# slp-rl/aero

Measured on NVIDIA H100. Metric: audio-seconds/sec forward, higher is better.
Workload: dtype f16 tensor-core operands and activation storage (10-bit mantissa = tf32), fp32 accumulate / norm inputs / cell state

## Files before the change

### aero_b200/csrc/tapgemm.cuh

```cuda
#pragma once
#include <cuda.h>
#include "common.cuh"

namespace aero {
struct TapGemmArgs {
    const void* a1;
    const void* a2;
    const void* w;
    const float* bias;
    const float* addend_fn;
    const float* colscale;
    const void* residual;
    const float* samp_affine;
    void* out;
    double* stats;
    aero_tapgemm_params p;
    int ntaps;
    int tiles_t;
    int ldw;
    int vec_a;
    int vec_o;
    int vec_o8;
    uint32_t dv_mul[3], dv_shr[3];
    int direct_f16;
    int direct_f32;
    int last_tile;
};
constexpr int kBM = 128;
constexpr int kMaxStages = 8;
constexpr int kMaxBN = 128;
constexpr int kEpiWarps = 8;
constexpr int kThreads = 128 + 32 * kEpiWarps;
constexpr int kATileBytes = kBM * 128;

struct TcShared {
    uint64_t full[kMaxStages];
    uint64_t empty[kMaxStages];
    float stats[kEpiWarps][8][2];
    float part[kEpiWarps][4][2];
    alignas(16) float stage[kEpiWarps][32][20];
};

using KernelFn = void (*)(CUtensorMap, CUtensorMap, CUtensorMap, TapGemmArgs, int, int, int);
int tapgemm_simt_launch(const TapGemmArgs& g, cudaStream_t st);
int tapgemm_tc_launch(const TapGemmArgs& g, cudaStream_t st);
bool tapgemm_tc_eligible(const aero_tapgemm_params& p);
}
```

### aero_b200/csrc/tapgemm_tc.cu

```cuda
#include <cuda.h>
#include <mutex>
#include <unordered_map>
#include <string>
#include <cstring>
#include <cstdlib>

#include "tapgemm.cuh"
#include "tc_common.cuh"

namespace aero {

KernelFn tapgemm_tc_kernels_bn32(bool f16a, bool f16o, int amode, bool res, bool stats);
KernelFn tapgemm_tc_kernels_bn64(bool f16a, bool f16o, int amode, bool res, bool stats);
KernelFn tapgemm_tc_kernels_bn96(bool f16a, bool f16o, int amode, bool res, bool stats);
KernelFn tapgemm_tc_kernels_bn128(bool f16a, bool f16o, int amode, bool res, bool stats);

typedef CUresult (*EncodeTiledFn)(CUtensorMap*, CUtensorMapDataType, cuuint32_t, void*, const cuuint64_t*, const cuuint64_t*,
                                  const cuuint32_t*, const cuuint32_t*, CUtensorMapInterleave, CUtensorMapSwizzle,
                                  CUtensorMapL2promotion, CUtensorMapFloatOOBfill);

static EncodeTiledFn get_encode() {
    static EncodeTiledFn fn = nullptr;
    static std::once_flag once;
    std::call_once(once, [] {
        void* p = nullptr;
        cudaDriverEntryPointQueryResult qres;
        if (cudaGetDriverEntryPoint("cuTensorMapEncodeTiled", &p, cudaEnableDefault, &qres) == cudaSuccess &&
            qres == cudaDriverEntryPointSuccess)
            fn = reinterpret_cast<EncodeTiledFn>(p);
    });
    return fn;
}

struct MapKey {
    const void* base;
    uint64_t d[4], s[3];
    uint32_t box[4], rank, swz, pad_;
    bool operator==(const MapKey& o) const { return std::memcmp(this, &o, sizeof(MapKey)) == 0; }
};
struct MapKeyHash {
    size_t operator()(const MapKey& k) const {
        const uint64_t* w = reinterpret_cast<const uint64_t*>(&k);
        size_t h = 1469598103934665603ull;
        for (size_t i = 0; i < sizeof(MapKey) / 8; ++i) h = (h ^ w[i]) * 1099511628211ull;
        return h;
    }
};

int encode_map(CUtensorMap* out, const void* base, uint32_t rank, const uint64_t* dims, const uint64_t* strides_bytes,
               const uint32_t* box, int swizzle_mode, int elem_bytes) {
    static std::mutex mu;
    static std::unordered_map<MapKey, CUtensorMap, MapKeyHash> cache;
    MapKey key;
    std::memset(&key, 0, sizeof(key));
    key.base = base;
    key.rank = rank;
    key.swz = (uint32_t)swizzle_mode | ((uint32_t)elem_bytes << 8);
    for (uint32_t i = 0; i < rank; ++i) { key.d[i] = dims[i]; key.box[i] = box[i]; }
    for (uint32_t i = 0; i + 1 < rank; ++i) key.s[i] = strides_bytes[i];
    {
        std::lock_guard<std::mutex> lk(mu);
        auto it = cache.find(key);
        if (it != cache.end()) { *out = it->second; return AERO_OK; }
    }
    EncodeTiledFn enc = get_encode();
    if (!enc) { set_error("cuTensorMapEncodeTiled not available from the driver"); return AERO_ERR_UNSUPPORTED; }
    cuuint64_t gd[4];
    cuuint64_t gs[3];
    cuuint32_t bx[4], es[4];
    for (uint32_t i = 0; i < rank; ++i) { gd[i] = dims[i]; bx[i] = box[i]; es[i] = 1; }
    for (uint32_t i = 0; i + 1 < rank; ++i) gs[i] = strides_bytes[i];
    CUresult r = enc(out, elem_bytes == 2 ? CU_TENSOR_MAP_DATA_TYPE_FLOAT16 : CU_TENSOR_MAP_DATA_TYPE_FLOAT32, rank, const_cast<void*>(base), gd, gs, bx, es,
                     CU_TENSOR_MAP_INTERLEAVE_NONE,
                     swizzle_mode == 2 ? CU_TENSOR_MAP_SWIZZLE_64B : CU_TENSOR_MAP_SWIZZLE_128B,
                     CU_TENSOR_MAP_L2_PROMOTION_L2_256B,
                     CU_TENSOR_MAP_FLOAT_OOB_FILL_NONE);
    if (r != CUDA_SUCCESS) {
        set_error("cuTensorMapEncodeTiled failed (%d): rank %u dims %llu %llu %llu %llu", (int)r, rank,
                  (unsigned long long)dims[0], (unsigned long long)dims[1], (unsigned long long)(rank > 2 ? dims[2] : 0),
                  (unsigned long long)(rank > 3 ? dims[3] : 0));
        return AERO_ERR_INVALID;
    }
    std::lock_guard<std::mutex> lk(mu);
    if (cache.size() > 4096) cache.clear();
    cache.emplace(key, *out);
    return AERO_OK;
}

static int pick_bn(int N) {
    const int ntiles = (N + kMaxBN - 1) / kMaxBN;
    const int per = (N + ntiles - 1) / ntiles;
    return (per + 31) & ~31;
}

static int tc_fixed_smem(int N, int BN) { return (int)sizeof(TcShared) + cdiv(N, BN) * BN * 4 + kBM * (BN + 4) * 4 + 1024; }
static int tc_stages(int N, int BN) {
    if (N > (1 << 20)) return 0;
    const int st = (227 * 1024 - tc_fixed_smem(N, BN)) / (kATileBytes + BN * 128);
    return st > kMaxStages ? kMaxStages : st;
}

bool tapgemm_tc_eligible(const aero_tapgemm_params& p) {
    const bool f16 = (p.flags & AERO_TG_A_F16) != 0;
    const int q = f16 ? 8 : 4;
    if (p.mode == AERO_TAPS_MIX)
        return p.w_sb == 0 && p.C1 % q == 0 && p.C2 == 0 && p.a1_st % q == 0 && p.a1_sb % q == 0 && p.N >= 8 &&
               p.stats_mode == 0 && !p.glu && p.F_out == 1 && p.F_in == 1 && tc_stages(p.N, pick_bn(p.N)) >= 2;
    if (p.w_sb != 0) return false;
    if (p.act == AERO_ACT_TANH) return false;
    if (p.act == AERO_ACT_LEAKY && (p.stats_mode != 0 || p.r_sb != 0 || p.r_sf != 0 || p.r_st != 0))
        return false;
    if (tc_stages(p.N, pick_bn(p.N)) < 2) return false;
    if (p.N < 8) return false;
    const int K = p.C1 + p.C2;
    if (K < 8 || (p.C1 % q) || (p.C2 % q)) return false;
    auto ok_strides = [q](int64_t sb, int64_t sf, int64_t st) { return sb % q == 0 && sf % q == 0 && st % q == 0 && st > 0; };
    if (p.C1 && !ok_strides(p.a1_sb, p.a1_sf, p.a1_st)) return false;
    if (p.C2 && !ok_strides(p.a2_sb, p.a2_sf, p.a2_st)) return false;
    if (p.stats_mode == 1) {
        const int Nout = p.glu ? p.N / 2 : p.N;
        if (p.groups < 1 || Nout % p.groups) return false;
        const int gw = Nout / p.groups;
        const int bn = pick_bn(p.N);
        if (gw % 8 || (p.glu ? bn / 2 : bn) / gw + 2 > 8) return false;
    }
    return true;
}

static int make_a_map(CUtensorMap* m, const void* base, int C, const aero_tapgemm_params& p, int64_t sb, int64_t sf, int64_t st, int esz) {
    uint64_t dims[4] = {(uint64_t)C, (uint64_t)p.T_in, (uint64_t)p.F_in, (uint64_t)p.B};
    int64_t s1 = st, s2 = sf, s3 = sb;
    if (s2 <= 0) s2 = s1 * p.T_in;
    if (s3 <= 0) s3 = s2 * p.F_in;
    uint64_t strides[3] = {(uint64_t)s1 * esz, (uint64_t)s2 * esz, (uint64_t)s3 * esz};
    uint32_t box[4] = {(uint32_t)(128 / esz), (uint32_t)kBM, 1, 1};
    return encode_map(m, base, 4, dims, strides, box, 0, esz);
}

struct TcKnobs {
    int direct_f32 = -1, direct_f16 = -1, stages = -1;
    TcKnobs() {
        auto rd = [](const char* name, int& v) { if (const char* e = getenv(name)) v = atoi(e); };
        rd("AERO_TC_DIRECT_F32", direct_f32); rd("AERO_TC_DIRECT_F16", direct_f16); rd("AERO_TC_STAGES", stages);
    }
};
static const TcKnobs& knobs() { static const TcKnobs k; return k; }

int tapgemm_tc_launch(const TapGemmArgs& g0, cudaStream_t st) {
    const TcKnobs& kn = knobs();
    TapGemmArgs g = g0;
    const aero_tapgemm_params& p = g.p;
    const bool f16a = p.precision == 2, f16o = (p.flags & AERO_TG_OUT_F16) != 0;
    const int esz = f16a ? 2 : 4, kBKc = 128 / esz;
    const int K = p.C1 + p.C2;
    const int BN = pick_bn(p.N);
    const int nslab = (p.mode == AERO_TAPS_CONVT) ? p.kf : p.kf * p.kt;
    CUtensorMap mA1, mA2, mW;
    int rc;
    const bool mix = p.mode == AERO_TAPS_MIX;
    if (mix) {
        uint64_t dims[3] = {(uint64_t)p.T, (uint64_t)p.C1, (uint64_t)p.B};
        uint64_t strides[2] = {(uint64_t)p.a1_st * esz, (uint64_t)(p.a1_sb > 0 ? p.a1_sb : (int64_t)p.a1_st * p.C1) * esz};
        uint32_t box[3] = {(uint32_t)(f16a ? 64 : 32), (uint32_t)kBKc, 1};
        if ((rc = encode_map(&mA1, g.a1, 3, dims, strides, box, 0, esz)) != AERO_OK) return rc;
    } else if (p.C1) { if ((rc = make_a_map(&mA1, g.a1, p.C1, p, p.a1_sb, p.a1_sf, p.a1_st, esz)) != AERO_OK) return rc; }
    if (p.C2) { if ((rc = make_a_map(&mA2, g.a2, p.C2, p, p.a2_sb, p.a2_sf, p.a2_st, esz)) != AERO_OK) return rc; }
    if (!p.C1) mA1 = mA2;
    if (!p.C2) mA2 = mA1;
    {
        const uint64_t npad = (uint64_t)((p.N + 3) & ~3);
        const uint64_t kp = f16a ? (uint64_t)((K + 7) & ~7) : (uint64_t)K;
        uint64_t dims[3] = {(uint64_t)K, npad, (uint64_t)nslab};
        uint64_t strides[2] = {kp * esz, kp * npad * esz};
        uint32_t box[3] = {(uint32_t)kBKc, (uint32_t)BN, 1};
        if ((rc = encode_map(&mW, g.w, 3, dims, strides, box, 0, esz)) != AERO_OK) return rc;
    }
    g.tiles_t = cdiv(p.T, kBM);
    g.direct_f32 = 0;
    g.direct_f16 = 2;
    if (kn.direct_f32 >= 0) g.direct_f32 = kn.direct_f32;
    if (kn.direct_f16 >= 0) g.direct_f16 = kn.direct_f16;
    const int64_t tiles = (int64_t)p.B * p.F_out * g.tiles_t;
    if (tiles > 2147483647LL) { set_error("aero_tapgemm_fwd: too many tiles"); return AERO_ERR_INVALID; }
    {
        const uint32_t divs[3] = {(uint32_t)cdiv(p.N, BN), (uint32_t)g.tiles_t, (uint32_t)p.F_out};
        for (int i = 0; i < 3; ++i) {
            uint32_t s = 0;
            while ((1ull << s) < divs[i]) ++s;
            const uint64_t two = 1ull << (31 + s);
            g.dv_mul[i] = (uint32_t)((two + divs[i] - 1) / divs[i]);
            g.dv_shr[i] = 31 + s;
        }
    }
    const int stage_bytes = kATileBytes + BN * 128;
    const int fixed = tc_fixed_smem(p.N, BN);
    int kStages = tc_stages(p.N, BN);
    if (kStages < 2) {
        set_error("aero_tapgemm_fwd(wgmma): N = %d leaves no shared memory for the pipeline", p.N);
        return AERO_ERR_UNSUPPORTED;
    }
    if (kn.stages >= 2 && kn.stages < kStages) kStages = kn.stages;
    const size_t smem = (size_t)kStages * stage_bytes + fixed;
    const int amode = p.glu ? 3 : (p.act == AERO_ACT_LEAKY ? 4 : p.act);
    if (p.glu && p.act != AERO_ACT_NONE) { set_error("aero_tapgemm_fwd(wgmma): GLU with an activation is not supported"); return AERO_ERR_UNSUPPORTED; }
    const bool res = g.residual != nullptr, stats = p.stats_mode != 0;
    const KernelFn kern = BN == 32 ? tapgemm_tc_kernels_bn32(f16a, f16o, amode, res, stats)
                        : BN == 64 ? tapgemm_tc_kernels_bn64(f16a, f16o, amode, res, stats)
                        : BN == 96 ? tapgemm_tc_kernels_bn96(f16a, f16o, amode, res, stats)
                                   : tapgemm_tc_kernels_bn128(f16a, f16o, amode, res, stats);
    if (!kern) {
        set_error("aero_tapgemm_fwd(wgmma): epilogue (act %d, residual %d, stats %d) is not built for operands %s / outputs %s",
                  amode, (int)res, (int)stats, f16a ? "f16" : "tf32", f16o ? "f16" : "f32");
        return AERO_ERR_UNSUPPORTED;
    }
    cudaFuncSetAttribute(kern, cudaFuncAttributeMaxDynamicSharedMemorySize, 227 * 1024);
    static int num_sms = 0;
    if (num_sms == 0) {
        int dev = 0;
        cudaGetDevice(&dev);
        cudaDeviceGetAttribute(&num_sms, cudaDevAttrMultiProcessorCount, dev);
    }
    const int n_tiles = cdiv(p.N, BN);
    const int64_t tiles_total = tiles * n_tiles;
    if (tiles_total > 2147483647LL) { set_error("aero_tapgemm_fwd: too many tiles"); return AERO_ERR_INVALID; }
    const int64_t want = num_sms;
    g.last_tile = (int)tiles_total - 1;
    dim3 grid((unsigned)(tiles_total < want ? tiles_total : want));
    kern<<<grid, kThreads, smem, st>>>(mA1, mA2, mW, g, kStages, n_tiles, (int)tiles_total);
    return check_launch("aero_tapgemm_fwd(wgmma)");
}

}
```

### aero_b200/csrc/tapgemm_tc_kernel.cuh

```cuda
#pragma once
#include <cuda.h>
#include <type_traits>

#include "tapgemm.cuh"
#include "tc_common.cuh"


namespace aero {

template <bool F16A> struct OperandKind { static constexpr int kBK = F16A ? 64 : 32; };

struct TapIter {
    int fi, dt, slab;
};
__device__ __forceinline__ bool tap_geometry(const aero_tapgemm_params& p, int tap, int fo, TapIter& it) {
    if (p.mode == AERO_TAPS_CONV) {
        const int jf = tap / p.kt, jt = tap - jf * p.kt;
        it.fi = fo * p.stride_f + jf - p.pad_f;
        it.dt = jt * p.dil_t - p.pad_t;
        it.slab = tap;
    } else {
        const int fof = fo + p.f_out_offset;
        it.fi = fof / p.stride_f - tap;
        it.dt = 0;
        it.slab = fof % p.stride_f + tap * p.stride_f;
    }
    return it.fi >= 0 && it.fi < p.F_in;
}

struct TileCoord {
    int b, fo, t0, n0, n_iters;
};
__device__ __forceinline__ int fast_div(int n, uint32_t mul, uint32_t shr) {
    return (int)(((uint64_t)(uint32_t)n * mul) >> shr);
}
__device__ __forceinline__ int valid_taps(const aero_tapgemm_params& p, int fo, int ntaps) {
    if (p.mode == AERO_TAPS_CONV) {
        const int base = fo * p.stride_f - p.pad_f;
        const int lo = max(0, -base), hi = min(p.kf - 1, p.F_in - 1 - base);
        return max(0, hi - lo + 1) * p.kt;
    }
    const int a = (fo + p.f_out_offset) / p.stride_f;
    const int lo = max(0, a - p.F_in + 1), hi = min(ntaps - 1, a);
    return max(0, hi - lo + 1);
}
__device__ __forceinline__ TileCoord tile_coord(const TapGemmArgs& g, int tile, int n_tiles, int BN, int nch1, int nch2) {
    const aero_tapgemm_params& p = g.p;
    TileCoord c;
    if (p.flags & AERO_TG_REVERSE) tile = g.last_tile - tile;
    const int mt = fast_div(tile, g.dv_mul[0], g.dv_shr[0]), nt = tile - mt * n_tiles;
    const int row = fast_div(mt, g.dv_mul[1], g.dv_shr[1]), tt = mt - row * g.tiles_t;
    c.b = fast_div(row, g.dv_mul[2], g.dv_shr[2]);
    c.fo = row - c.b * p.F_out;
    c.t0 = tt * kBM;
    c.n0 = nt * BN;
    c.n_iters = (p.mode == AERO_TAPS_MIX) ? nch1 : valid_taps(p, c.fo, g.ntaps) * (nch1 + nch2);
    return c;
}

template <int AMODE>
__device__ __forceinline__ void epilogue_stage_a(const uint32_t (&r)[16], uint32_t stg_row, uint32_t sbias) {
    float4 bv[4];
#pragma unroll
    for (int j = 0; j < 4; ++j) bv[j] = lds128(sbias + 16 * j);
#pragma unroll
    for (int j = 0; j < 16; j += 4) {
        float v[4] = {__uint_as_float(r[j]) + bv[j / 4].x, __uint_as_float(r[j + 1]) + bv[j / 4].y,
                      __uint_as_float(r[j + 2]) + bv[j / 4].z, __uint_as_float(r[j + 3]) + bv[j / 4].w};
#pragma unroll
        for (int u = 0; u < 4; ++u) {
            if (AMODE == 1) v[u] = gelu_exact(v[u]);
            else if (AMODE == 2) v[u] = fmaxf(v[u], 0.f);
            else if (AMODE == 4) v[u] = leaky_f(v[u]);
        }
        if (AMODE == 3) {
            sts64(stg_row + (j / 2) * 4, v[0] * sigmoid_f(v[1]), v[2] * sigmoid_f(v[3]));
        } else {
            sts128(stg_row + j * 4, make_float4(v[0], v[1], v[2], v[3]));
        }
    }
}

template <int AMODE, bool RES, bool STATS, typename TO>
__device__ __forceinline__ void epilogue_fast_tile(TcShared* sh, const TapGemmArgs& g, const TileCoord& tc, uint32_t tacc, int BN, int q,
                                                   int ew, int lane, int Nout, int gw, int c_start, int c_step, uint32_t sbias) {
    const aero_tapgemm_params& p = g.p;
    constexpr int CNT = (AMODE == 3) ? 8 : 16;
    constexpr int LPR = CNT / 4;
    constexpr int RPI = 32 / LPR;
    const uint32_t stg = smem_u32(&sh->stage[ew][0][0]);
    const bool rnd = (p.flags & 1) && sizeof(TO) == 4;
    float sa = 1.f, sb = 0.f;
    if (g.samp_affine) { sa = g.samp_affine[2 * tc.b]; sb = g.samp_affine[2 * tc.b + 1]; }
    const int cq = lane % LPR, ro = lane / LPR;
    const int row0 = tc.t0 + q * 32;
    const int rows = min(32, p.T - row0);
    const int g_lo = ((AMODE == 3) ? tc.n0 >> 1 : tc.n0) / gw;
    TO* const obase = static_cast<TO*>(g.out) + (int64_t)tc.b * p.o_sb + (int64_t)tc.fo * p.o_sf + (int64_t)row0 * p.o_st;
    const TO* const rbase = RES ? static_cast<const TO*>(g.residual) + (int64_t)tc.b * p.r_sb + (int64_t)tc.fo * p.r_sf + (int64_t)row0 * p.r_st : nullptr;
    const float* const adp = g.addend_fn ? g.addend_fn + (int64_t)tc.fo * Nout : nullptr;
    for (int c0 = c_start; c0 < BN; c0 += c_step) {
        const int nb = tc.n0 + c0;
        if (nb >= p.N) break;
        uint32_t r[16];
        if (tc.n_iters > 0) {
            acc_ld16(tacc + 4u * (uint32_t)c0, r);
        } else {
#pragma unroll
            for (int j = 0; j < 16; ++j) r[j] = 0u;
        }
        epilogue_stage_a<AMODE>(r, stg + (uint32_t)lane * 80u, sbias + (uint32_t)nb * 4u);
        __syncwarp();
        const int no0 = (AMODE == 3) ? nb >> 1 : nb;
        const int nn = no0 + 4 * cq;
        float ls = 0.f, lq = 0.f;
        if (nn < Nout) {
            float4 ad = make_float4(0.f, 0.f, 0.f, 0.f);
            const bool has_ad = adp != nullptr, affine = g.samp_affine != nullptr;
            if (has_ad) ad = *reinterpret_cast<const float4*>(adp + nn);
            uint32_t sp = stg + (uint32_t)(ro * 80 + cq * 16);
            TO* op = obase + (int64_t)ro * p.o_st + nn;
            const TO* rp = RES ? rbase + (int64_t)ro * p.r_st + nn : nullptr;
            const int64_t ostep = (int64_t)RPI * p.o_st, rstep = (int64_t)RPI * p.r_st;
#pragma unroll 2
            for (int rr = ro; rr < rows; rr += RPI) {
                float4 x = lds128(sp);
                sp += RPI * 80;
                if (has_ad) { x.x += ad.x; x.y += ad.y; x.z += ad.z; x.w += ad.w; }
                if (RES) {
                    const float4 rs = ld4(rp);
                    x.x += rs.x; x.y += rs.y; x.z += rs.z; x.w += rs.w;
                    rp += rstep;
                }
                if (affine) { x.x = fmaf(x.x, sa, sb); x.y = fmaf(x.y, sa, sb); x.z = fmaf(x.z, sa, sb); x.w = fmaf(x.w, sa, sb); }
                if (rnd) { x.x = round_tf32_rna(x.x); x.y = round_tf32_rna(x.y); x.z = round_tf32_rna(x.z); x.w = round_tf32_rna(x.w); }
                if (STATS) {
                    if (sizeof(TO) == 2) {
                        x.x = stored(x.x, op); x.y = stored(x.y, op); x.z = stored(x.z, op); x.w = stored(x.w, op);
                    }
                    ls += (x.x + x.y) + (x.z + x.w);
                    lq += (x.x * x.x + x.y * x.y) + (x.z * x.z + x.w * x.w);
                }
                st4(op, x);
                op += ostep;
            }
        }
        if (STATS) {
            const int g_first = no0 / gw, g_last = (min(no0 + CNT, Nout) - 1) / gw;
            if (g_first == g_last) {
                const float a = warp_sum(ls), c = warp_sum(lq);
                if (lane == 0) { sh->stats[ew][g_first - g_lo][0] += a; sh->stats[ew][g_first - g_lo][1] += c; }
            } else {
                for (int o = LPR; o < 32; o <<= 1) { ls += __shfl_xor_sync(0xffffffffu, ls, o); lq += __shfl_xor_sync(0xffffffffu, lq, o); }
                if (lane < LPR) { sh->part[ew][lane][0] = ls; sh->part[ew][lane][1] = lq; }
                __syncwarp();
                if (lane == 0) {
                    for (int u = 0; u < LPR; ++u) {
                        const int nq = no0 + 4 * u;
                        if (nq < Nout) {
                            sh->stats[ew][nq / gw - g_lo][0] += sh->part[ew][u][0];
                            sh->stats[ew][nq / gw - g_lo][1] += sh->part[ew][u][1];
                        }
                    }
                }
            }
        }
        __syncwarp();
    }
}

template <int AMODE, bool RES, bool STATS, typename TO>
__device__ __forceinline__ void epilogue_direct(TcShared* sh, const TapGemmArgs& g, const TileCoord& tc, uint32_t tacc, int BN, int q, int ew,
                                                int lane, int Nout, int gw, int c_start, int c_step, uint32_t sbias) {
    const aero_tapgemm_params& p = g.p;
    constexpr int CNT = (AMODE == 3) ? 8 : 16;
    constexpr bool F16 = sizeof(TO) == 2;
    const int t = tc.t0 + q * 32 + lane;
    const bool row_ok = t < p.T;
    TO* const orow = static_cast<TO*>(g.out) + (int64_t)tc.b * p.o_sb + (int64_t)tc.fo * p.o_sf + (int64_t)t * p.o_st;
    const TO* const rrow = RES ? static_cast<const TO*>(g.residual) + (int64_t)tc.b * p.r_sb + (int64_t)tc.fo * p.r_sf + (int64_t)t * p.r_st : nullptr;
    const float* const adp = g.addend_fn ? g.addend_fn + (int64_t)tc.fo * Nout : nullptr;
    float sa = 1.f, sb = 0.f;
    const bool affine = g.samp_affine != nullptr;
    if (affine) { sa = g.samp_affine[2 * tc.b]; sb = g.samp_affine[2 * tc.b + 1]; }
    const bool rnd = (p.flags & 1) && !F16;
    const int g_lo = ((AMODE == 3) ? tc.n0 >> 1 : tc.n0) / gw;
    int cur_g = -1;
    float ssum = 0.f, ssq = 0.f;
    for (int c0 = c_start; c0 < BN; c0 += c_step) {
        const int nb = tc.n0 + c0;
        if (nb >= p.N) break;
        uint32_t r[16];
        if (tc.n_iters > 0) {
            acc_ld16(tacc + 4u * (uint32_t)c0, r);
        } else {
#pragma unroll
            for (int j = 0; j < 16; ++j) r[j] = 0u;
        }
        float v[16];
#pragma unroll
        for (int j = 0; j < 16; ++j) v[j] = __uint_as_float(r[j]);
        {
            float4 bv[4];
#pragma unroll
            for (int j = 0; j < 4; ++j) bv[j] = lds128(sbias + (uint32_t)nb * 4u + 16u * j);
#pragma unroll
            for (int j = 0; j < 4; ++j) { v[4 * j] += bv[j].x; v[4 * j + 1] += bv[j].y; v[4 * j + 2] += bv[j].z; v[4 * j + 3] += bv[j].w; }
        }
        float o[CNT];
        if (AMODE == 3) {
#pragma unroll
            for (int j = 0; j < 8; ++j) o[j] = v[2 * j] * sigmoid_f(v[2 * j + 1]);
        } else {
#pragma unroll
            for (int j = 0; j < 16; ++j)
                o[j] = (AMODE == 1) ? gelu_exact(v[j]) : (AMODE == 2) ? fmaxf(v[j], 0.f) : (AMODE == 4) ? leaky_f(v[j]) : v[j];
        }
        const int no0 = (AMODE == 3) ? nb >> 1 : nb;
        const int n_ok = min(CNT, Nout - no0);
        if (row_ok) {
            if (adp) {
#pragma unroll
                for (int j = 0; j < CNT; j += 4)
                    if (j < n_ok) {
                        const float4 a = __ldg(reinterpret_cast<const float4*>(adp + no0 + j));
                        o[j] += a.x; o[j + 1] += a.y; o[j + 2] += a.z; o[j + 3] += a.w;
                    }
            }
            if (RES) {
#pragma unroll
                for (int j = 0; j < CNT; j += 4)
                    if (j < n_ok) {
                        const float4 a = ld4(rrow + no0 + j);
                        o[j] += a.x; o[j + 1] += a.y; o[j + 2] += a.z; o[j + 3] += a.w;
                    }
            }
            if (affine) {
#pragma unroll
                for (int j = 0; j < CNT; ++j) o[j] = fmaf(o[j], sa, sb);
            }
            if (rnd) {
#pragma unroll
                for (int j = 0; j < CNT; ++j) o[j] = round_tf32_rna(o[j]);
            }
            if (F16 && STATS) {
#pragma unroll
                for (int j = 0; j < CNT; ++j) o[j] = stored(o[j], orow);
            }
            if (F16) {
#pragma unroll
                for (int j = 0; j < CNT; j += 8)
                    if (j < n_ok) {
                        uint4 u;
                        u.x = pack_half2_sat(o[j], o[j + 1]); u.y = pack_half2_sat(o[j + 2], o[j + 3]);
                        u.z = pack_half2_sat(o[j + 4], o[j + 5]); u.w = pack_half2_sat(o[j + 6], o[j + 7]);
                        *reinterpret_cast<uint4*>(orow + no0 + j) = u;
                    }
            } else {
#pragma unroll
                for (int j = 0; j < CNT; j += 4)
                    if (j < n_ok) *reinterpret_cast<float4*>(orow + no0 + j) = make_float4(o[j], o[j + 1], o[j + 2], o[j + 3]);
            }
        }
        if (STATS) {
#pragma unroll
            for (int j = 0; j < CNT; j += 4) {
                if (j < n_ok) {
                    const int gi = (no0 + j) / gw;
                    if (gi != cur_g) {
                        if (cur_g >= 0) {
                            const float a = warp_sum(ssum), c = warp_sum(ssq);
                            if (lane == 0) { sh->stats[ew][cur_g - g_lo][0] += a; sh->stats[ew][cur_g - g_lo][1] += c; }
                        }
                        cur_g = gi; ssum = 0.f; ssq = 0.f;
                    }
                    if (row_ok) {
                        ssum += (o[j] + o[j + 1]) + (o[j + 2] + o[j + 3]);
                        ssq += (o[j] * o[j] + o[j + 1] * o[j + 1]) + (o[j + 2] * o[j + 2] + o[j + 3] * o[j + 3]);
                    }
                }
            }
        }
    }
    if (STATS && cur_g >= 0) {
        const float a = warp_sum(ssum), c = warp_sum(ssq);
        if (lane == 0) { sh->stats[ew][cur_g - g_lo][0] += a; sh->stats[ew][cur_g - g_lo][1] += c; }
    }
}

template <int BN, bool F16A>
__device__ __forceinline__ void tile_mainloop(TcShared* sh, uint8_t* smem, int& stage, uint32_t& phase, const int kStages, const int stage_bytes,
                                              const int n_iters, const bool mix, const int wg, float* acc, const int ldacc) {
    float d[BN / 2];
    const int tid = threadIdx.x & 127, wl = tid >> 5, lane = tid & 31;
    int prev = -1;
    for (int i = 0; i < n_iters; ++i) {
        mbar_wait(&sh->full[stage], phase);
        const uint32_t sa = smem_u32(smem + stage * stage_bytes);
        const uint64_t db = make_desc_sw128(sa + kATileBytes);
        wgmma_fence();
        if (mix && F16A) {
            if constexpr (F16A) {
                const uint32_t sw = sa + (uint32_t)wg * 8192u;
                const uint64_t da = (uint64_t)((sw >> 4) & 0x3FFF) | ((uint64_t)(8192 >> 4) << 16) | ((uint64_t)(1024 >> 4) << 32) | ((uint64_t)1 << 62);
#pragma unroll
                for (int k = 0; k < 4; ++k) Wgmma<BN, true, 1>::ss(d, da + (uint64_t)(k * (2048 >> 4)), db + 2 * k, (i > 0 || k > 0) ? 1u : 0u);
            }
        } else if (mix) {
            if constexpr (!F16A) {
                const int m = wg * 64 + wl * 16 + (lane >> 2), c = lane & 3;
#pragma unroll
                for (int k = 0; k < 4; ++k) {
                    uint32_t a[4];
#pragma unroll
                    for (int u = 0; u < 4; ++u) {
                        const int mm = m + (u & 1) * 8, kk = 8 * k + c + (u >> 1) * 4;
                        const uint32_t addr = sa + (uint32_t)((mm >> 5) * 4096 + kk * 128 + ((((mm & 31) >> 2) ^ (kk & 7)) << 4) + ((mm & 3) << 2));
                        asm volatile("ld.shared.b32 %0, [%1];" : "=r"(a[u]) : "r"(addr));
                    }
                    Wgmma<BN, false, 0>::rs(d, a, db + 2 * k, (i > 0 || k > 0) ? 1u : 0u);
                }
            }
        } else {
            const uint64_t da = make_desc_sw128(sa + (uint32_t)wg * (64 * 128));
#pragma unroll
            for (int k = 0; k < 4; ++k)
                Wgmma<BN, F16A, 0>::ss(d, da + 2 * k, db + 2 * k, (i > 0 || k > 0) ? 1u : 0u);
        }
        wgmma_commit();
        wgmma_wait<1>();
        if (prev >= 0 && tid == 0) mbar_arrive(&sh->empty[prev]);
        prev = stage;
        if (++stage == kStages) { stage = 0; phase ^= 1; }
    }
    wgmma_wait<0>();
    if (prev >= 0 && tid == 0) mbar_arrive(&sh->empty[prev]);
    float* row = acc + (wg * 64 + wl * 16 + (lane >> 2)) * ldacc + 2 * (lane & 3);
#pragma unroll
    for (int j = 0; j < BN / 8; ++j) {
        *reinterpret_cast<float2*>(row + 8 * j) = make_float2(d[4 * j], d[4 * j + 1]);
        *reinterpret_cast<float2*>(row + 8 * ldacc + 8 * j) = make_float2(d[4 * j + 2], d[4 * j + 3]);
    }
}

template <int BN, int AMODE, bool RES, bool STATS, bool F16A, bool F16O>
__global__ void __launch_bounds__(kThreads, 1)
tapgemm_tc_kernel(const __grid_constant__ CUtensorMap mapA1, const __grid_constant__ CUtensorMap mapA2,
                  const __grid_constant__ CUtensorMap mapW, const TapGemmArgs g, const int kStages, const int n_tiles,
                  const int tiles_total) {
    extern __shared__ uint8_t smem_raw[];
    uint8_t* smem = reinterpret_cast<uint8_t*>((reinterpret_cast<uintptr_t>(smem_raw) + 1023) & ~(uintptr_t)1023);
    constexpr int stage_bytes = kATileBytes + BN * 128;
    TcShared* sh = reinterpret_cast<TcShared*>(smem + kStages * stage_bytes);
    float* const sbias_f = reinterpret_cast<float*>(sh + 1);
    const uint32_t sbias = smem_u32(sbias_f);
    float* const acc = sbias_f + n_tiles * BN;
    constexpr int ldacc = BN + 4;

    using TO = typename std::conditional<F16O, __half, float>::type;
    constexpr int kBKc = OperandKind<F16A>::kBK;
    const aero_tapgemm_params& p = g.p;
    const int warp = threadIdx.x >> 5, lane = threadIdx.x & 31;
    const int nch1 = (p.C1 + kBKc - 1) / kBKc, nch2 = (p.C2 + kBKc - 1) / kBKc;
    const bool mix = p.mode == AERO_TAPS_MIX;

    for (int i = threadIdx.x; i < n_tiles * BN; i += kThreads) sbias_f[i] = (g.bias && i < g.p.N) ? g.bias[i] : 0.f;
    if (threadIdx.x == 0) {
        for (int s = 0; s < kStages; ++s) { mbar_init(&sh->full[s], 1); mbar_init(&sh->empty[s], 2); }
        asm volatile("fence.mbarrier_init.release.cluster;" ::: "memory");
        for (int w = 0; w < kEpiWarps; ++w)
            for (int i = 0; i < 8; ++i) { sh->stats[w][i][0] = 0.f; sh->stats[w][i][1] = 0.f; }
    }
    __syncthreads();

    if (warp == 0) {
        if (lane == 0) {
            asm volatile("prefetch.tensormap [%0];" ::"l"(&mapA1) : "memory");
            asm volatile("prefetch.tensormap [%0];" ::"l"(&mapW) : "memory");
            int stage = 0;
            uint32_t phase = 0;
            const uint32_t tx = (uint32_t)stage_bytes;
            int ptl = 0;
            for (int tile = blockIdx.x; tile < tiles_total; tile += gridDim.x, ++ptl) {
                const TileCoord c = tile_coord(g, tile, n_tiles, BN, nch1, nch2);
                if (mix) {
                    for (int kc = 0; kc < nch1; ++kc) {
                        mbar_wait(&sh->empty[stage], phase ^ 1);
                        uint8_t* sa = smem + stage * stage_bytes;
                        mbar_expect_tx(&sh->full[stage], tx);
                        constexpr int kBoxM = F16A ? 64 : 32;
#pragma unroll
                        for (int j = 0; j < 128 / kBoxM; ++j)
                            tma_load_3d(sa + j * (kATileBytes / (128 / kBoxM)), &mapA1, &sh->full[stage], c.t0 + kBoxM * j, kc * kBKc, c.b);
                        tma_load_3d(sa + kATileBytes, &mapW, &sh->full[stage], kc * kBKc, c.n0, 0);
                        if (++stage == kStages) { stage = 0; phase ^= 1; }
                    }
                    continue;
                }
                for (int tap = 0; tap < g.ntaps; ++tap) {
                    TapIter it;
                    if (!tap_geometry(p, tap, c.fo, it)) continue;
                    for (int src = 0; src < 2; ++src) {
                        const int nch = src ? nch2 : nch1;
                        const CUtensorMap* mA = src ? &mapA2 : &mapA1;
                        const int kw0 = src ? p.C1 : 0;
                        for (int kc = 0; kc < nch; ++kc) {
                            mbar_wait(&sh->empty[stage], phase ^ 1);
                            uint8_t* sa = smem + stage * stage_bytes;
                            mbar_expect_tx(&sh->full[stage], tx);
                            tma_load_4d(sa, mA, &sh->full[stage], kc * kBKc, c.t0 + it.dt, it.fi, c.b);
                            tma_load_3d(sa + kATileBytes, &mapW, &sh->full[stage], kw0 + kc * kBKc, c.n0, it.slab);
                            if (++stage == kStages) { stage = 0; phase ^= 1; }
                        }
                    }
                }
            }
        }
    } else if (warp >= 4) {
        const int wg = (warp >> 2) - 1;
        const int ew = warp - 4;
        const int q = 2 * wg + (warp & 1);
        const int grp = (warp >> 1) & 1;
        const int m = q * 32 + lane;
        const int Nout = p.glu ? p.N / 2 : p.N;
        const int gw = (p.stats_mode == 1) ? Nout / p.groups : Nout;
        const bool rnd = (p.flags & 1) && !F16O;
        const int c_start = grp * 16, c_step = 32;
        const bool fast = !mix && g.vec_o && !g.colscale && (p.stats_mode == 0 || gw % 4 == 0);
        int stage = 0, local = 0;
        uint32_t phase = 0;
        for (int tile = blockIdx.x; tile < tiles_total; tile += gridDim.x, ++local) {
            const TileCoord tc = tile_coord(g, tile, n_tiles, BN, nch1, nch2);
            const int b = tc.b, fo = tc.fo, t0 = tc.t0, n0 = tc.n0, n_iters = tc.n_iters;
            tile_mainloop<BN, F16A>(sh, smem, stage, phase, kStages, stage_bytes, n_iters, mix, wg, acc, ldacc);
            warpgroup_sync(1 + wg);
            const uint32_t tacc = smem_u32(acc + m * ldacc);
            const int t = t0 + m;
            const bool row_ok = t < p.T;
            float sa = 1.f, sb = 0.f;
            if (g.samp_affine) { sa = g.samp_affine[2 * b]; sb = g.samp_affine[2 * b + 1]; }
            TO* op = static_cast<TO*>(g.out) + (int64_t)b * p.o_sb + (int64_t)fo * p.o_sf + (int64_t)t * p.o_st;
            const TO* rp = g.residual ? static_cast<const TO*>(g.residual) + (int64_t)b * p.r_sb + (int64_t)fo * p.r_sf + (int64_t)t * p.r_st : nullptr;
            const float* csp = g.colscale ? g.colscale + (int64_t)b * p.cs_sb + (int64_t)t * p.cs_st : nullptr;
            const float* adp = g.addend_fn ? g.addend_fn + (int64_t)fo * Nout : nullptr;
            int cur_g = -1;
            float ssum = 0.f, ssq = 0.f;
            const int g_lo = (p.glu ? n0 >> 1 : n0) / gw;

            if (mix) {
                const float gate = (row_ok && g.colscale) ? g.colscale[(int64_t)b * p.cs_sb + t] : 1.f;
                TO* ob = static_cast<TO*>(g.out) + (int64_t)b * p.o_sb + t;
                for (int c0 = c_start; c0 < BN; c0 += c_step) {
                    uint32_t r[16];
                    acc_ld16(tacc + 4u * (uint32_t)c0, r);
                    if (row_ok) {
#pragma unroll
                        for (int j = 0; j < 16; ++j) {
                            const int n = n0 + c0 + j;
                            if (n < p.N) {
                                float x = __uint_as_float(r[j]) * gate;
                                if (rnd) x = round_tf32_rna(x);
                                stf(ob + (int64_t)n * p.o_st, x);
                            }
                        }
                    }
                }
            } else if (fast && (F16O ? (g.vec_o8 && (g.direct_f16 == 1 || (g.direct_f16 == 2 && AMODE == 3))) : g.direct_f32)) {
                epilogue_direct<AMODE, RES, STATS, TO>(sh, g, tc, tacc, BN, q, ew, lane, Nout, gw, c_start, c_step, sbias);
            } else if (fast) {
                epilogue_fast_tile<AMODE, RES, STATS, TO>(sh, g, tc, tacc, BN, q, ew, lane, Nout, gw, c_start, c_step, sbias);
            } else {
                for (int c0 = 0; c0 < (grp == 0 ? BN : 0); c0 += 16) {
                    uint32_t r[16];
                    if (n_iters > 0) {
                        acc_ld16(tacc + 4u * (uint32_t)c0, r);
                    } else {
#pragma unroll
                        for (int j = 0; j < 16; ++j) r[j] = 0u;
                    }
                    const int nb = n0 + c0;
                    if (nb >= p.N) continue;
                    float v[16];
#pragma unroll
                    for (int j = 0; j < 16; ++j) {
                        const int n = nb + j;
                        float x = __uint_as_float(r[j]);
                        if (row_ok && n < p.N) {
                            x += sbias_f[n];
                            if (csp) x *= csp[n];
                            if (p.act == AERO_ACT_GELU) x = gelu_exact(x);
                            else if (p.act == AERO_ACT_RELU) x = fmaxf(x, 0.f);
                            else if (AMODE == 4) x = leaky_f(x);
                        }
                        v[j] = x;
                    }
                    float o[16];
                    int no0, cnt;
                    if (p.glu) {
                        no0 = nb >> 1;
                        cnt = 8;
#pragma unroll
                        for (int j = 0; j < 8; ++j) o[j] = v[2 * j] * sigmoid_f(v[2 * j + 1]);
                    } else {
                        no0 = nb;
                        cnt = 16;
#pragma unroll
                        for (int j = 0; j < 16; ++j) o[j] = v[j];
                    }
#pragma unroll
                    for (int sub = 0; sub < 2; ++sub) {
                        if (sub * 8 >= cnt) break;
                        const int ns = no0 + sub * 8;
                        if (p.stats_mode != 0 && ns < Nout) {
                            const int gi = ns / gw;
                            if (gi != cur_g) {
                                if (cur_g >= 0) {
                                    const float a = warp_sum(ssum), c = warp_sum(ssq);
                                    if (lane == 0) { sh->stats[ew][cur_g - g_lo][0] = a; sh->stats[ew][cur_g - g_lo][1] = c; }
                                }
                                cur_g = gi; ssum = 0.f; ssq = 0.f;
                            }
                        }
#pragma unroll
                        for (int j = 0; j < 8; ++j) {
                            const int jj = sub * 8 + j;
                            const int nn = no0 + jj;
                            if (row_ok && nn < Nout) {
                                float x = o[jj];
                                if (adp) x += adp[nn];
                                if (rp) x += ldf(rp + nn);
                                x = x * sa + sb;
                                if (rnd) x = round_tf32_rna(x);
                                x = stored(x, op);
                                o[jj] = x;
                                ssum += x;
                                ssq += x * x;
                            }
                        }
                    }
                    if (row_ok) {
#pragma unroll
                        for (int j = 0; j < 16; ++j)
                            if (j < cnt && no0 + j < Nout) stf(op + no0 + j, o[j]);
                    }
                }
                if (p.stats_mode != 0 && cur_g >= 0) {
                    const float a = warp_sum(ssum), c = warp_sum(ssq);
                    if (lane == 0) { sh->stats[ew][cur_g - g_lo][0] = a; sh->stats[ew][cur_g - g_lo][1] = c; }
                }
            }
            warpgroup_sync(1 + wg);
            if (p.stats_mode != 0) {
                __syncwarp();
                if (lane < 8) {
                    const float a = sh->stats[ew][lane][0], c = sh->stats[ew][lane][1];
                    const int gi = g_lo + lane;
                    const int ngroups = (p.stats_mode == 1) ? p.groups : 1;
                    if (gi < ngroups && (a != 0.f || c != 0.f)) {
                        const int64_t slot = (p.stats_mode == 1) ? ((int64_t)b * p.groups + gi) : ((int64_t)b * p.F_out + fo);
                        atomicAdd(&g.stats[2 * slot], (double)a);
                        atomicAdd(&g.stats[2 * slot + 1], (double)c);
                    }
                    sh->stats[ew][lane][0] = 0.f;
                    sh->stats[ew][lane][1] = 0.f;
                }
                __syncwarp();
            }
        }
    }
}



template <int BN, bool F16A, bool F16O>
static KernelFn pick_kernel(int amode, bool res, bool stats) {
#define AERO_TC_K(A, R, S) tapgemm_tc_kernel<BN, A, R, S, F16A, F16O>
    if (amode == 4) return (res || stats) ? nullptr : AERO_TC_K(4, false, false);
    if constexpr (!F16A && !F16O) {
        static const KernelFn table[4][2][2] = {
            {{AERO_TC_K(0, false, false), AERO_TC_K(0, false, true)}, {AERO_TC_K(0, true, false), AERO_TC_K(0, true, true)}},
            {{AERO_TC_K(1, false, false), AERO_TC_K(1, false, true)}, {AERO_TC_K(1, true, false), AERO_TC_K(1, true, true)}},
            {{AERO_TC_K(2, false, false), AERO_TC_K(2, false, true)}, {AERO_TC_K(2, true, false), AERO_TC_K(2, true, true)}},
            {{AERO_TC_K(3, false, false), AERO_TC_K(3, false, true)}, {AERO_TC_K(3, true, false), AERO_TC_K(3, true, true)}}};
        return table[amode][res][stats];
    } else if constexpr (F16O) {
        if (stats) return (amode == 0 && !res) ? AERO_TC_K(0, false, true) : nullptr;
        if (res) return amode == 0 ? AERO_TC_K(0, true, false) : nullptr;
        switch (amode) {
            case 0: return AERO_TC_K(0, false, false);
            case 1: return AERO_TC_K(1, false, false);
            case 2: return AERO_TC_K(2, false, false);
            default: return AERO_TC_K(3, false, false);
        }
    } else {
        if (res) return nullptr;
        if (stats) return amode == 0 ? AERO_TC_K(0, false, true) : nullptr;
        switch (amode) {
            case 0: return AERO_TC_K(0, false, false);
            case 1: return AERO_TC_K(1, false, false);
            case 2: return AERO_TC_K(2, false, false);
            default: return AERO_TC_K(3, false, false);
        }
    }
#undef AERO_TC_K
}

template <int BN>
static KernelFn pick_kernel_bn(bool f16a, bool f16o, int amode, bool res, bool stats) {
    return f16a ? (f16o ? pick_kernel<BN, true, true>(amode, res, stats) : pick_kernel<BN, true, false>(amode, res, stats))
                : (f16o ? pick_kernel<BN, false, true>(amode, res, stats) : pick_kernel<BN, false, false>(amode, res, stats));
}

}
```

### aero_b200/csrc/wgmma.cuh

```cuda
#pragma once
#include <cstdint>

namespace aero {

__device__ __forceinline__ void wgmma_fence() { asm volatile("wgmma.fence.sync.aligned;" ::: "memory"); }
__device__ __forceinline__ void wgmma_commit() { asm volatile("wgmma.commit_group.sync.aligned;" ::: "memory"); }
template <int PENDING>
__device__ __forceinline__ void wgmma_wait() { asm volatile("wgmma.wait_group.sync.aligned %0;" ::"n"(PENDING) : "memory"); }

template <int ROWB>
__device__ __forceinline__ uint64_t make_desc_kmajor(uint32_t saddr) {
    return (uint64_t)((saddr >> 4) & 0x3FFF) | ((uint64_t)1 << 16) | ((uint64_t)((ROWB * 8) >> 4) << 32) |
           ((uint64_t)(ROWB == 128 ? 1 : 2) << 62);
}
__device__ __forceinline__ uint64_t make_desc_sw128(uint32_t saddr) { return make_desc_kmajor<128>(saddr); }

template <int N, bool F16, int TA> struct Wgmma;

template <int TA> struct Wgmma<16, true, TA> {
    static __device__ __forceinline__ void ss(float (&d)[8], uint64_t da, uint64_t db, uint32_t acc) {
        asm volatile("{\n\t.reg .pred p;\n\tsetp.ne.b32 p, %10, 0;\n\t"
                     "wgmma.mma_async.sync.aligned.m64n16k16.f32.f16.f16 {%0, %1, %2, %3, %4, %5, %6, %7}, %8, %9, p, 1, 1, %11, 0;\n\t}"
            : "+f"(d[0]), "+f"(d[1]), "+f"(d[2]), "+f"(d[3]), "+f"(d[4]), "+f"(d[5]), "+f"(d[6]), "+f"(d[7])
            : "l"(da), "l"(db), "r"(acc), "n"(TA));
    }
};
template <> struct Wgmma<16, false, 0> {
    static __device__ __forceinline__ void ss(float (&d)[8], uint64_t da, uint64_t db, uint32_t acc) {
        asm volatile("{\n\t.reg .pred p;\n\tsetp.ne.b32 p, %10, 0;\n\t"
                     "wgmma.mma_async.sync.aligned.m64n16k8.f32.tf32.tf32 {%0, %1, %2, %3, %4, %5, %6, %7}, %8, %9, p, 1, 1;\n\t}"
            : "+f"(d[0]), "+f"(d[1]), "+f"(d[2]), "+f"(d[3]), "+f"(d[4]), "+f"(d[5]), "+f"(d[6]), "+f"(d[7])
            : "l"(da), "l"(db), "r"(acc));
    }
    static __device__ __forceinline__ void rs(float (&d)[8], const uint32_t (&a)[4], uint64_t db, uint32_t acc) {
        asm volatile("{\n\t.reg .pred p;\n\tsetp.ne.b32 p, %13, 0;\n\t"
                     "wgmma.mma_async.sync.aligned.m64n16k8.f32.tf32.tf32 {%0, %1, %2, %3, %4, %5, %6, %7}, {%8, %9, %10, %11}, %12, p, 1, 1;\n\t}"
            : "+f"(d[0]), "+f"(d[1]), "+f"(d[2]), "+f"(d[3]), "+f"(d[4]), "+f"(d[5]), "+f"(d[6]), "+f"(d[7])
            : "r"(a[0]), "r"(a[1]), "r"(a[2]), "r"(a[3]), "l"(db), "r"(acc));
    }
};

template <int TA> struct Wgmma<32, true, TA> {
    static __device__ __forceinline__ void ss(float (&d)[16], uint64_t da, uint64_t db, uint32_t acc) {
        asm volatile("{\n\t.reg .pred p;\n\tsetp.ne.b32 p, %18, 0;\n\t"
                     "wgmma.mma_async.sync.aligned.m64n32k16.f32.f16.f16 {%0, %1, %2, %3, %4, %5, %6, %7, %8, %9, %10, %11, %12, %13, %14, %15}, %16, %17, p, 1, 1, %19, 0;\n\t}"
            : "+f"(d[0]), "+f"(d[1]), "+f"(d[2]), "+f"(d[3]), "+f"(d[4]), "+f"(d[5]), "+f"(d[6]), "+f"(d[7]),
              "+f"(d[8]), "+f"(d[9]), "+f"(d[10]), "+f"(d[11]), "+f"(d[12]), "+f"(d[13]), "+f"(d[14]), "+f"(d[15])
            : "l"(da), "l"(db), "r"(acc), "n"(TA));
    }
};
template <> struct Wgmma<32, false, 0> {
    static __device__ __forceinline__ void ss(float (&d)[16], uint64_t da, uint64_t db, uint32_t acc) {
        asm volatile("{\n\t.reg .pred p;\n\tsetp.ne.b32 p, %18, 0;\n\t"
                     "wgmma.mma_async.sync.aligned.m64n32k8.f32.tf32.tf32 {%0, %1, %2, %3, %4, %5, %6, %7, %8, %9, %10, %11, %12, %13, %14, %15}, %16, %17, p, 1, 1;\n\t}"
            : "+f"(d[0]), "+f"(d[1]), "+f"(d[2]), "+f"(d[3]), "+f"(d[4]), "+f"(d[5]), "+f"(d[6]), "+f"(d[7]),
              "+f"(d[8]), "+f"(d[9]), "+f"(d[10]), "+f"(d[11]), "+f"(d[12]), "+f"(d[13]), "+f"(d[14]), "+f"(d[15])
            : "l"(da), "l"(db), "r"(acc));
    }
    static __device__ __forceinline__ void rs(float (&d)[16], const uint32_t (&a)[4], uint64_t db, uint32_t acc) {
        asm volatile("{\n\t.reg .pred p;\n\tsetp.ne.b32 p, %21, 0;\n\t"
                     "wgmma.mma_async.sync.aligned.m64n32k8.f32.tf32.tf32 {%0, %1, %2, %3, %4, %5, %6, %7, %8, %9, %10, %11, %12, %13, %14, %15}, {%16, %17, %18, %19}, %20, p, 1, 1;\n\t}"
            : "+f"(d[0]), "+f"(d[1]), "+f"(d[2]), "+f"(d[3]), "+f"(d[4]), "+f"(d[5]), "+f"(d[6]), "+f"(d[7]),
              "+f"(d[8]), "+f"(d[9]), "+f"(d[10]), "+f"(d[11]), "+f"(d[12]), "+f"(d[13]), "+f"(d[14]), "+f"(d[15])
            : "r"(a[0]), "r"(a[1]), "r"(a[2]), "r"(a[3]), "l"(db), "r"(acc));
    }
};

template <int TA> struct Wgmma<48, true, TA> {
    static __device__ __forceinline__ void ss(float (&d)[24], uint64_t da, uint64_t db, uint32_t acc) {
        asm volatile("{\n\t.reg .pred p;\n\tsetp.ne.b32 p, %26, 0;\n\t"
                     "wgmma.mma_async.sync.aligned.m64n48k16.f32.f16.f16 {%0, %1, %2, %3, %4, %5, %6, %7, %8, %9, %10, %11, %12, %13, %14, %15, %16, %17, %18, %19, %20, %21, %22, %23}, %24, %25, p, 1, 1, %27, 0;\n\t}"
            : "+f"(d[0]), "+f"(d[1]), "+f"(d[2]), "+f"(d[3]), "+f"(d[4]), "+f"(d[5]), "+f"(d[6]), "+f"(d[7]),
              "+f"(d[8]), "+f"(d[9]), "+f"(d[10]), "+f"(d[11]), "+f"(d[12]), "+f"(d[13]), "+f"(d[14]), "+f"(d[15]),
              "+f"(d[16]), "+f"(d[17]), "+f"(d[18]), "+f"(d[19]), "+f"(d[20]), "+f"(d[21]), "+f"(d[22]), "+f"(d[23])
            : "l"(da), "l"(db), "r"(acc), "n"(TA));
    }
};
template <> struct Wgmma<48, false, 0> {
    static __device__ __forceinline__ void ss(float (&d)[24], uint64_t da, uint64_t db, uint32_t acc) {
        asm volatile("{\n\t.reg .pred p;\n\tsetp.ne.b32 p, %26, 0;\n\t"
                     "wgmma.mma_async.sync.aligned.m64n48k8.f32.tf32.tf32 {%0, %1, %2, %3, %4, %5, %6, %7, %8, %9, %10, %11, %12, %13, %14, %15, %16, %17, %18, %19, %20, %21, %22, %23}, %24, %25, p, 1, 1;\n\t}"
            : "+f"(d[0]), "+f"(d[1]), "+f"(d[2]), "+f"(d[3]), "+f"(d[4]), "+f"(d[5]), "+f"(d[6]), "+f"(d[7]),
              "+f"(d[8]), "+f"(d[9]), "+f"(d[10]), "+f"(d[11]), "+f"(d[12]), "+f"(d[13]), "+f"(d[14]), "+f"(d[15]),
              "+f"(d[16]), "+f"(d[17]), "+f"(d[18]), "+f"(d[19]), "+f"(d[20]), "+f"(d[21]), "+f"(d[22]), "+f"(d[23])
            : "l"(da), "l"(db), "r"(acc));
    }
    static __device__ __forceinline__ void rs(float (&d)[24], const uint32_t (&a)[4], uint64_t db, uint32_t acc) {
        asm volatile("{\n\t.reg .pred p;\n\tsetp.ne.b32 p, %29, 0;\n\t"
                     "wgmma.mma_async.sync.aligned.m64n48k8.f32.tf32.tf32 {%0, %1, %2, %3, %4, %5, %6, %7, %8, %9, %10, %11, %12, %13, %14, %15, %16, %17, %18, %19, %20, %21, %22, %23}, {%24, %25, %26, %27}, %28, p, 1, 1;\n\t}"
            : "+f"(d[0]), "+f"(d[1]), "+f"(d[2]), "+f"(d[3]), "+f"(d[4]), "+f"(d[5]), "+f"(d[6]), "+f"(d[7]),
              "+f"(d[8]), "+f"(d[9]), "+f"(d[10]), "+f"(d[11]), "+f"(d[12]), "+f"(d[13]), "+f"(d[14]), "+f"(d[15]),
              "+f"(d[16]), "+f"(d[17]), "+f"(d[18]), "+f"(d[19]), "+f"(d[20]), "+f"(d[21]), "+f"(d[22]), "+f"(d[23])
            : "r"(a[0]), "r"(a[1]), "r"(a[2]), "r"(a[3]), "l"(db), "r"(acc));
    }
};

template <int TA> struct Wgmma<64, true, TA> {
    static __device__ __forceinline__ void ss(float (&d)[32], uint64_t da, uint64_t db, uint32_t acc) {
        asm volatile("{\n\t.reg .pred p;\n\tsetp.ne.b32 p, %34, 0;\n\t"
                     "wgmma.mma_async.sync.aligned.m64n64k16.f32.f16.f16 {%0, %1, %2, %3, %4, %5, %6, %7, %8, %9, %10, %11, %12, %13, %14, %15, %16, %17, %18, %19, %20, %21, %22, %23, %24, %25, %26, %27, %28, %29, %30, %31}, %32, %33, p, 1, 1, %35, 0;\n\t}"
            : "+f"(d[0]), "+f"(d[1]), "+f"(d[2]), "+f"(d[3]), "+f"(d[4]), "+f"(d[5]), "+f"(d[6]), "+f"(d[7]),
              "+f"(d[8]), "+f"(d[9]), "+f"(d[10]), "+f"(d[11]), "+f"(d[12]), "+f"(d[13]), "+f"(d[14]), "+f"(d[15]),
              "+f"(d[16]), "+f"(d[17]), "+f"(d[18]), "+f"(d[19]), "+f"(d[20]), "+f"(d[21]), "+f"(d[22]), "+f"(d[23]),
              "+f"(d[24]), "+f"(d[25]), "+f"(d[26]), "+f"(d[27]), "+f"(d[28]), "+f"(d[29]), "+f"(d[30]), "+f"(d[31])
            : "l"(da), "l"(db), "r"(acc), "n"(TA));
    }
};
template <> struct Wgmma<64, false, 0> {
    static __device__ __forceinline__ void ss(float (&d)[32], uint64_t da, uint64_t db, uint32_t acc) {
        asm volatile("{\n\t.reg .pred p;\n\tsetp.ne.b32 p, %34, 0;\n\t"
                     "wgmma.mma_async.sync.aligned.m64n64k8.f32.tf32.tf32 {%0, %1, %2, %3, %4, %5, %6, %7, %8, %9, %10, %11, %12, %13, %14, %15, %16, %17, %18, %19, %20, %21, %22, %23, %24, %25, %26, %27, %28, %29, %30, %31}, %32, %33, p, 1, 1;\n\t}"
            : "+f"(d[0]), "+f"(d[1]), "+f"(d[2]), "+f"(d[3]), "+f"(d[4]), "+f"(d[5]), "+f"(d[6]), "+f"(d[7]),
              "+f"(d[8]), "+f"(d[9]), "+f"(d[10]), "+f"(d[11]), "+f"(d[12]), "+f"(d[13]), "+f"(d[14]), "+f"(d[15]),
              "+f"(d[16]), "+f"(d[17]), "+f"(d[18]), "+f"(d[19]), "+f"(d[20]), "+f"(d[21]), "+f"(d[22]), "+f"(d[23]),
              "+f"(d[24]), "+f"(d[25]), "+f"(d[26]), "+f"(d[27]), "+f"(d[28]), "+f"(d[29]), "+f"(d[30]), "+f"(d[31])
            : "l"(da), "l"(db), "r"(acc));
    }
    static __device__ __forceinline__ void rs(float (&d)[32], const uint32_t (&a)[4], uint64_t db, uint32_t acc) {
        asm volatile("{\n\t.reg .pred p;\n\tsetp.ne.b32 p, %37, 0;\n\t"
                     "wgmma.mma_async.sync.aligned.m64n64k8.f32.tf32.tf32 {%0, %1, %2, %3, %4, %5, %6, %7, %8, %9, %10, %11, %12, %13, %14, %15, %16, %17, %18, %19, %20, %21, %22, %23, %24, %25, %26, %27, %28, %29, %30, %31}, {%32, %33, %34, %35}, %36, p, 1, 1;\n\t}"
            : "+f"(d[0]), "+f"(d[1]), "+f"(d[2]), "+f"(d[3]), "+f"(d[4]), "+f"(d[5]), "+f"(d[6]), "+f"(d[7]),
              "+f"(d[8]), "+f"(d[9]), "+f"(d[10]), "+f"(d[11]), "+f"(d[12]), "+f"(d[13]), "+f"(d[14]), "+f"(d[15]),
              "+f"(d[16]), "+f"(d[17]), "+f"(d[18]), "+f"(d[19]), "+f"(d[20]), "+f"(d[21]), "+f"(d[22]), "+f"(d[23]),
              "+f"(d[24]), "+f"(d[25]), "+f"(d[26]), "+f"(d[27]), "+f"(d[28]), "+f"(d[29]), "+f"(d[30]), "+f"(d[31])
            : "r"(a[0]), "r"(a[1]), "r"(a[2]), "r"(a[3]), "l"(db), "r"(acc));
    }
};

template <int TA> struct Wgmma<80, true, TA> {
    static __device__ __forceinline__ void ss(float (&d)[40], uint64_t da, uint64_t db, uint32_t acc) {
        asm volatile("{\n\t.reg .pred p;\n\tsetp.ne.b32 p, %42, 0;\n\t"
                     "wgmma.mma_async.sync.aligned.m64n80k16.f32.f16.f16 {%0, %1, %2, %3, %4, %5, %6, %7, %8, %9, %10, %11, %12, %13, %14, %15, %16, %17, %18, %19, %20, %21, %22, %23, %24, %25, %26, %27, %28, %29, %30, %31, %32, %33, %34, %35, %36, %37, %38, %39}, %40, %41, p, 1, 1, %43, 0;\n\t}"
            : "+f"(d[0]), "+f"(d[1]), "+f"(d[2]), "+f"(d[3]), "+f"(d[4]), "+f"(d[5]), "+f"(d[6]), "+f"(d[7]),
              "+f"(d[8]), "+f"(d[9]), "+f"(d[10]), "+f"(d[11]), "+f"(d[12]), "+f"(d[13]), "+f"(d[14]), "+f"(d[15]),
              "+f"(d[16]), "+f"(d[17]), "+f"(d[18]), "+f"(d[19]), "+f"(d[20]), "+f"(d[21]), "+f"(d[22]), "+f"(d[23]),
              "+f"(d[24]), "+f"(d[25]), "+f"(d[26]), "+f"(d[27]), "+f"(d[28]), "+f"(d[29]), "+f"(d[30]), "+f"(d[31]),
              "+f"(d[32]), "+f"(d[33]), "+f"(d[34]), "+f"(d[35]), "+f"(d[36]), "+f"(d[37]), "+f"(d[38]), "+f"(d[39])
            : "l"(da), "l"(db), "r"(acc), "n"(TA));
    }
};
template <> struct Wgmma<80, false, 0> {
    static __device__ __forceinline__ void ss(float (&d)[40], uint64_t da, uint64_t db, uint32_t acc) {
        asm volatile("{\n\t.reg .pred p;\n\tsetp.ne.b32 p, %42, 0;\n\t"
                     "wgmma.mma_async.sync.aligned.m64n80k8.f32.tf32.tf32 {%0, %1, %2, %3, %4, %5, %6, %7, %8, %9, %10, %11, %12, %13, %14, %15, %16, %17, %18, %19, %20, %21, %22, %23, %24, %25, %26, %27, %28, %29, %30, %31, %32, %33, %34, %35, %36, %37, %38, %39}, %40, %41, p, 1, 1;\n\t}"
            : "+f"(d[0]), "+f"(d[1]), "+f"(d[2]), "+f"(d[3]), "+f"(d[4]), "+f"(d[5]), "+f"(d[6]), "+f"(d[7]),
              "+f"(d[8]), "+f"(d[9]), "+f"(d[10]), "+f"(d[11]), "+f"(d[12]), "+f"(d[13]), "+f"(d[14]), "+f"(d[15]),
              "+f"(d[16]), "+f"(d[17]), "+f"(d[18]), "+f"(d[19]), "+f"(d[20]), "+f"(d[21]), "+f"(d[22]), "+f"(d[23]),
              "+f"(d[24]), "+f"(d[25]), "+f"(d[26]), "+f"(d[27]), "+f"(d[28]), "+f"(d[29]), "+f"(d[30]), "+f"(d[31]),
              "+f"(d[32]), "+f"(d[33]), "+f"(d[34]), "+f"(d[35]), "+f"(d[36]), "+f"(d[37]), "+f"(d[38]), "+f"(d[39])
            : "l"(da), "l"(db), "r"(acc));
    }
    static __device__ __forceinline__ void rs(float (&d)[40], const uint32_t (&a)[4], uint64_t db, uint32_t acc) {
        asm volatile("{\n\t.reg .pred p;\n\tsetp.ne.b32 p, %45, 0;\n\t"
                     "wgmma.mma_async.sync.aligned.m64n80k8.f32.tf32.tf32 {%0, %1, %2, %3, %4, %5, %6, %7, %8, %9, %10, %11, %12, %13, %14, %15, %16, %17, %18, %19, %20, %21, %22, %23, %24, %25, %26, %27, %28, %29, %30, %31, %32, %33, %34, %35, %36, %37, %38, %39}, {%40, %41, %42, %43}, %44, p, 1, 1;\n\t}"
            : "+f"(d[0]), "+f"(d[1]), "+f"(d[2]), "+f"(d[3]), "+f"(d[4]), "+f"(d[5]), "+f"(d[6]), "+f"(d[7]),
              "+f"(d[8]), "+f"(d[9]), "+f"(d[10]), "+f"(d[11]), "+f"(d[12]), "+f"(d[13]), "+f"(d[14]), "+f"(d[15]),
              "+f"(d[16]), "+f"(d[17]), "+f"(d[18]), "+f"(d[19]), "+f"(d[20]), "+f"(d[21]), "+f"(d[22]), "+f"(d[23]),
              "+f"(d[24]), "+f"(d[25]), "+f"(d[26]), "+f"(d[27]), "+f"(d[28]), "+f"(d[29]), "+f"(d[30]), "+f"(d[31]),
              "+f"(d[32]), "+f"(d[33]), "+f"(d[34]), "+f"(d[35]), "+f"(d[36]), "+f"(d[37]), "+f"(d[38]), "+f"(d[39])
            : "r"(a[0]), "r"(a[1]), "r"(a[2]), "r"(a[3]), "l"(db), "r"(acc));
    }
};

template <int TA> struct Wgmma<96, true, TA> {
    static __device__ __forceinline__ void ss(float (&d)[48], uint64_t da, uint64_t db, uint32_t acc) {
        asm volatile("{\n\t.reg .pred p;\n\tsetp.ne.b32 p, %50, 0;\n\t"
                     "wgmma.mma_async.sync.aligned.m64n96k16.f32.f16.f16 {%0, %1, %2, %3, %4, %5, %6, %7, %8, %9, %10, %11, %12, %13, %14, %15, %16, %17, %18, %19, %20, %21, %22, %23, %24, %25, %26, %27, %28, %29, %30, %31, %32, %33, %34, %35, %36, %37, %38, %39, %40, %41, %42, %43, %44, %45, %46, %47}, %48, %49, p, 1, 1, %51, 0;\n\t}"
            : "+f"(d[0]), "+f"(d[1]), "+f"(d[2]), "+f"(d[3]), "+f"(d[4]), "+f"(d[5]), "+f"(d[6]), "+f"(d[7]),
              "+f"(d[8]), "+f"(d[9]), "+f"(d[10]), "+f"(d[11]), "+f"(d[12]), "+f"(d[13]), "+f"(d[14]), "+f"(d[15]),
              "+f"(d[16]), "+f"(d[17]), "+f"(d[18]), "+f"(d[19]), "+f"(d[20]), "+f"(d[21]), "+f"(d[22]), "+f"(d[23]),
              "+f"(d[24]), "+f"(d[25]), "+f"(d[26]), "+f"(d[27]), "+f"(d[28]), "+f"(d[29]), "+f"(d[30]), "+f"(d[31]),
              "+f"(d[32]), "+f"(d[33]), "+f"(d[34]), "+f"(d[35]), "+f"(d[36]), "+f"(d[37]), "+f"(d[38]), "+f"(d[39]),
              "+f"(d[40]), "+f"(d[41]), "+f"(d[42]), "+f"(d[43]), "+f"(d[44]), "+f"(d[45]), "+f"(d[46]), "+f"(d[47])
            : "l"(da), "l"(db), "r"(acc), "n"(TA));
    }
};
template <> struct Wgmma<96, false, 0> {
    static __device__ __forceinline__ void ss(float (&d)[48], uint64_t da, uint64_t db, uint32_t acc) {
        asm volatile("{\n\t.reg .pred p;\n\tsetp.ne.b32 p, %50, 0;\n\t"
                     "wgmma.mma_async.sync.aligned.m64n96k8.f32.tf32.tf32 {%0, %1, %2, %3, %4, %5, %6, %7, %8, %9, %10, %11, %12, %13, %14, %15, %16, %17, %18, %19, %20, %21, %22, %23, %24, %25, %26, %27, %28, %29, %30, %31, %32, %33, %34, %35, %36, %37, %38, %39, %40, %41, %42, %43, %44, %45, %46, %47}, %48, %49, p, 1, 1;\n\t}"
            : "+f"(d[0]), "+f"(d[1]), "+f"(d[2]), "+f"(d[3]), "+f"(d[4]), "+f"(d[5]), "+f"(d[6]), "+f"(d[7]),
              "+f"(d[8]), "+f"(d[9]), "+f"(d[10]), "+f"(d[11]), "+f"(d[12]), "+f"(d[13]), "+f"(d[14]), "+f"(d[15]),
              "+f"(d[16]), "+f"(d[17]), "+f"(d[18]), "+f"(d[19]), "+f"(d[20]), "+f"(d[21]), "+f"(d[22]), "+f"(d[23]),
              "+f"(d[24]), "+f"(d[25]), "+f"(d[26]), "+f"(d[27]), "+f"(d[28]), "+f"(d[29]), "+f"(d[30]), "+f"(d[31]),
              "+f"(d[32]), "+f"(d[33]), "+f"(d[34]), "+f"(d[35]), "+f"(d[36]), "+f"(d[37]), "+f"(d[38]), "+f"(d[39]),
              "+f"(d[40]), "+f"(d[41]), "+f"(d[42]), "+f"(d[43]), "+f"(d[44]), "+f"(d[45]), "+f"(d[46]), "+f"(d[47])
            : "l"(da), "l"(db), "r"(acc));
    }
    static __device__ __forceinline__ void rs(float (&d)[48], const uint32_t (&a)[4], uint64_t db, uint32_t acc) {
        asm volatile("{\n\t.reg .pred p;\n\tsetp.ne.b32 p, %53, 0;\n\t"
                     "wgmma.mma_async.sync.aligned.m64n96k8.f32.tf32.tf32 {%0, %1, %2, %3, %4, %5, %6, %7, %8, %9, %10, %11, %12, %13, %14, %15, %16, %17, %18, %19, %20, %21, %22, %23, %24, %25, %26, %27, %28, %29, %30, %31, %32, %33, %34, %35, %36, %37, %38, %39, %40, %41, %42, %43, %44, %45, %46, %47}, {%48, %49, %50, %51}, %52, p, 1, 1;\n\t}"
            : "+f"(d[0]), "+f"(d[1]), "+f"(d[2]), "+f"(d[3]), "+f"(d[4]), "+f"(d[5]), "+f"(d[6]), "+f"(d[7]),
              "+f"(d[8]), "+f"(d[9]), "+f"(d[10]), "+f"(d[11]), "+f"(d[12]), "+f"(d[13]), "+f"(d[14]), "+f"(d[15]),
              "+f"(d[16]), "+f"(d[17]), "+f"(d[18]), "+f"(d[19]), "+f"(d[20]), "+f"(d[21]), "+f"(d[22]), "+f"(d[23]),
              "+f"(d[24]), "+f"(d[25]), "+f"(d[26]), "+f"(d[27]), "+f"(d[28]), "+f"(d[29]), "+f"(d[30]), "+f"(d[31]),
              "+f"(d[32]), "+f"(d[33]), "+f"(d[34]), "+f"(d[35]), "+f"(d[36]), "+f"(d[37]), "+f"(d[38]), "+f"(d[39]),
              "+f"(d[40]), "+f"(d[41]), "+f"(d[42]), "+f"(d[43]), "+f"(d[44]), "+f"(d[45]), "+f"(d[46]), "+f"(d[47])
            : "r"(a[0]), "r"(a[1]), "r"(a[2]), "r"(a[3]), "l"(db), "r"(acc));
    }
};

template <int TA> struct Wgmma<112, true, TA> {
    static __device__ __forceinline__ void ss(float (&d)[56], uint64_t da, uint64_t db, uint32_t acc) {
        asm volatile("{\n\t.reg .pred p;\n\tsetp.ne.b32 p, %58, 0;\n\t"
                     "wgmma.mma_async.sync.aligned.m64n112k16.f32.f16.f16 {%0, %1, %2, %3, %4, %5, %6, %7, %8, %9, %10, %11, %12, %13, %14, %15, %16, %17, %18, %19, %20, %21, %22, %23, %24, %25, %26, %27, %28, %29, %30, %31, %32, %33, %34, %35, %36, %37, %38, %39, %40, %41, %42, %43, %44, %45, %46, %47, %48, %49, %50, %51, %52, %53, %54, %55}, %56, %57, p, 1, 1, %59, 0;\n\t}"
            : "+f"(d[0]), "+f"(d[1]), "+f"(d[2]), "+f"(d[3]), "+f"(d[4]), "+f"(d[5]), "+f"(d[6]), "+f"(d[7]),
              "+f"(d[8]), "+f"(d[9]), "+f"(d[10]), "+f"(d[11]), "+f"(d[12]), "+f"(d[13]), "+f"(d[14]), "+f"(d[15]),
              "+f"(d[16]), "+f"(d[17]), "+f"(d[18]), "+f"(d[19]), "+f"(d[20]), "+f"(d[21]), "+f"(d[22]), "+f"(d[23]),
              "+f"(d[24]), "+f"(d[25]), "+f"(d[26]), "+f"(d[27]), "+f"(d[28]), "+f"(d[29]), "+f"(d[30]), "+f"(d[31]),
              "+f"(d[32]), "+f"(d[33]), "+f"(d[34]), "+f"(d[35]), "+f"(d[36]), "+f"(d[37]), "+f"(d[38]), "+f"(d[39]),
              "+f"(d[40]), "+f"(d[41]), "+f"(d[42]), "+f"(d[43]), "+f"(d[44]), "+f"(d[45]), "+f"(d[46]), "+f"(d[47]),
              "+f"(d[48]), "+f"(d[49]), "+f"(d[50]), "+f"(d[51]), "+f"(d[52]), "+f"(d[53]), "+f"(d[54]), "+f"(d[55])
            : "l"(da), "l"(db), "r"(acc), "n"(TA));
    }
};
template <> struct Wgmma<112, false, 0> {
    static __device__ __forceinline__ void ss(float (&d)[56], uint64_t da, uint64_t db, uint32_t acc) {
        asm volatile("{\n\t.reg .pred p;\n\tsetp.ne.b32 p, %58, 0;\n\t"
                     "wgmma.mma_async.sync.aligned.m64n112k8.f32.tf32.tf32 {%0, %1, %2, %3, %4, %5, %6, %7, %8, %9, %10, %11, %12, %13, %14, %15, %16, %17, %18, %19, %20, %21, %22, %23, %24, %25, %26, %27, %28, %29, %30, %31, %32, %33, %34, %35, %36, %37, %38, %39, %40, %41, %42, %43, %44, %45, %46, %47, %48, %49, %50, %51, %52, %53, %54, %55}, %56, %57, p, 1, 1;\n\t}"
            : "+f"(d[0]), "+f"(d[1]), "+f"(d[2]), "+f"(d[3]), "+f"(d[4]), "+f"(d[5]), "+f"(d[6]), "+f"(d[7]),
              "+f"(d[8]), "+f"(d[9]), "+f"(d[10]), "+f"(d[11]), "+f"(d[12]), "+f"(d[13]), "+f"(d[14]), "+f"(d[15]),
              "+f"(d[16]), "+f"(d[17]), "+f"(d[18]), "+f"(d[19]), "+f"(d[20]), "+f"(d[21]), "+f"(d[22]), "+f"(d[23]),
              "+f"(d[24]), "+f"(d[25]), "+f"(d[26]), "+f"(d[27]), "+f"(d[28]), "+f"(d[29]), "+f"(d[30]), "+f"(d[31]),
              "+f"(d[32]), "+f"(d[33]), "+f"(d[34]), "+f"(d[35]), "+f"(d[36]), "+f"(d[37]), "+f"(d[38]), "+f"(d[39]),
              "+f"(d[40]), "+f"(d[41]), "+f"(d[42]), "+f"(d[43]), "+f"(d[44]), "+f"(d[45]), "+f"(d[46]), "+f"(d[47]),
              "+f"(d[48]), "+f"(d[49]), "+f"(d[50]), "+f"(d[51]), "+f"(d[52]), "+f"(d[53]), "+f"(d[54]), "+f"(d[55])
            : "l"(da), "l"(db), "r"(acc));
    }
    static __device__ __forceinline__ void rs(float (&d)[56], const uint32_t (&a)[4], uint64_t db, uint32_t acc) {
        asm volatile("{\n\t.reg .pred p;\n\tsetp.ne.b32 p, %61, 0;\n\t"
                     "wgmma.mma_async.sync.aligned.m64n112k8.f32.tf32.tf32 {%0, %1, %2, %3, %4, %5, %6, %7, %8, %9, %10, %11, %12, %13, %14, %15, %16, %17, %18, %19, %20, %21, %22, %23, %24, %25, %26, %27, %28, %29, %30, %31, %32, %33, %34, %35, %36, %37, %38, %39, %40, %41, %42, %43, %44, %45, %46, %47, %48, %49, %50, %51, %52, %53, %54, %55}, {%56, %57, %58, %59}, %60, p, 1, 1;\n\t}"
            : "+f"(d[0]), "+f"(d[1]), "+f"(d[2]), "+f"(d[3]), "+f"(d[4]), "+f"(d[5]), "+f"(d[6]), "+f"(d[7]),
              "+f"(d[8]), "+f"(d[9]), "+f"(d[10]), "+f"(d[11]), "+f"(d[12]), "+f"(d[13]), "+f"(d[14]), "+f"(d[15]),
              "+f"(d[16]), "+f"(d[17]), "+f"(d[18]), "+f"(d[19]), "+f"(d[20]), "+f"(d[21]), "+f"(d[22]), "+f"(d[23]),
              "+f"(d[24]), "+f"(d[25]), "+f"(d[26]), "+f"(d[27]), "+f"(d[28]), "+f"(d[29]), "+f"(d[30]), "+f"(d[31]),
              "+f"(d[32]), "+f"(d[33]), "+f"(d[34]), "+f"(d[35]), "+f"(d[36]), "+f"(d[37]), "+f"(d[38]), "+f"(d[39]),
              "+f"(d[40]), "+f"(d[41]), "+f"(d[42]), "+f"(d[43]), "+f"(d[44]), "+f"(d[45]), "+f"(d[46]), "+f"(d[47]),
              "+f"(d[48]), "+f"(d[49]), "+f"(d[50]), "+f"(d[51]), "+f"(d[52]), "+f"(d[53]), "+f"(d[54]), "+f"(d[55])
            : "r"(a[0]), "r"(a[1]), "r"(a[2]), "r"(a[3]), "l"(db), "r"(acc));
    }
};

template <int TA> struct Wgmma<128, true, TA> {
    static __device__ __forceinline__ void ss(float (&d)[64], uint64_t da, uint64_t db, uint32_t acc) {
        asm volatile("{\n\t.reg .pred p;\n\tsetp.ne.b32 p, %66, 0;\n\t"
                     "wgmma.mma_async.sync.aligned.m64n128k16.f32.f16.f16 {%0, %1, %2, %3, %4, %5, %6, %7, %8, %9, %10, %11, %12, %13, %14, %15, %16, %17, %18, %19, %20, %21, %22, %23, %24, %25, %26, %27, %28, %29, %30, %31, %32, %33, %34, %35, %36, %37, %38, %39, %40, %41, %42, %43, %44, %45, %46, %47, %48, %49, %50, %51, %52, %53, %54, %55, %56, %57, %58, %59, %60, %61, %62, %63}, %64, %65, p, 1, 1, %67, 0;\n\t}"
            : "+f"(d[0]), "+f"(d[1]), "+f"(d[2]), "+f"(d[3]), "+f"(d[4]), "+f"(d[5]), "+f"(d[6]), "+f"(d[7]),
              "+f"(d[8]), "+f"(d[9]), "+f"(d[10]), "+f"(d[11]), "+f"(d[12]), "+f"(d[13]), "+f"(d[14]), "+f"(d[15]),
              "+f"(d[16]), "+f"(d[17]), "+f"(d[18]), "+f"(d[19]), "+f"(d[20]), "+f"(d[21]), "+f"(d[22]), "+f"(d[23]),
              "+f"(d[24]), "+f"(d[25]), "+f"(d[26]), "+f"(d[27]), "+f"(d[28]), "+f"(d[29]), "+f"(d[30]), "+f"(d[31]),
              "+f"(d[32]), "+f"(d[33]), "+f"(d[34]), "+f"(d[35]), "+f"(d[36]), "+f"(d[37]), "+f"(d[38]), "+f"(d[39]),
              "+f"(d[40]), "+f"(d[41]), "+f"(d[42]), "+f"(d[43]), "+f"(d[44]), "+f"(d[45]), "+f"(d[46]), "+f"(d[47]),
              "+f"(d[48]), "+f"(d[49]), "+f"(d[50]), "+f"(d[51]), "+f"(d[52]), "+f"(d[53]), "+f"(d[54]), "+f"(d[55]),
              "+f"(d[56]), "+f"(d[57]), "+f"(d[58]), "+f"(d[59]), "+f"(d[60]), "+f"(d[61]), "+f"(d[62]), "+f"(d[63])
            : "l"(da), "l"(db), "r"(acc), "n"(TA));
    }
};
template <> struct Wgmma<128, false, 0> {
    static __device__ __forceinline__ void ss(float (&d)[64], uint64_t da, uint64_t db, uint32_t acc) {
        asm volatile("{\n\t.reg .pred p;\n\tsetp.ne.b32 p, %66, 0;\n\t"
                     "wgmma.mma_async.sync.aligned.m64n128k8.f32.tf32.tf32 {%0, %1, %2, %3, %4, %5, %6, %7, %8, %9, %10, %11, %12, %13, %14, %15, %16, %17, %18, %19, %20, %21, %22, %23, %24, %25, %26, %27, %28, %29, %30, %31, %32, %33, %34, %35, %36, %37, %38, %39, %40, %41, %42, %43, %44, %45, %46, %47, %48, %49, %50, %51, %52, %53, %54, %55, %56, %57, %58, %59, %60, %61, %62, %63}, %64, %65, p, 1, 1;\n\t}"
            : "+f"(d[0]), "+f"(d[1]), "+f"(d[2]), "+f"(d[3]), "+f"(d[4]), "+f"(d[5]), "+f"(d[6]), "+f"(d[7]),
              "+f"(d[8]), "+f"(d[9]), "+f"(d[10]), "+f"(d[11]), "+f"(d[12]), "+f"(d[13]), "+f"(d[14]), "+f"(d[15]),
              "+f"(d[16]), "+f"(d[17]), "+f"(d[18]), "+f"(d[19]), "+f"(d[20]), "+f"(d[21]), "+f"(d[22]), "+f"(d[23]),
              "+f"(d[24]), "+f"(d[25]), "+f"(d[26]), "+f"(d[27]), "+f"(d[28]), "+f"(d[29]), "+f"(d[30]), "+f"(d[31]),
              "+f"(d[32]), "+f"(d[33]), "+f"(d[34]), "+f"(d[35]), "+f"(d[36]), "+f"(d[37]), "+f"(d[38]), "+f"(d[39]),
              "+f"(d[40]), "+f"(d[41]), "+f"(d[42]), "+f"(d[43]), "+f"(d[44]), "+f"(d[45]), "+f"(d[46]), "+f"(d[47]),
              "+f"(d[48]), "+f"(d[49]), "+f"(d[50]), "+f"(d[51]), "+f"(d[52]), "+f"(d[53]), "+f"(d[54]), "+f"(d[55]),
              "+f"(d[56]), "+f"(d[57]), "+f"(d[58]), "+f"(d[59]), "+f"(d[60]), "+f"(d[61]), "+f"(d[62]), "+f"(d[63])
            : "l"(da), "l"(db), "r"(acc));
    }
    static __device__ __forceinline__ void rs(float (&d)[64], const uint32_t (&a)[4], uint64_t db, uint32_t acc) {
        asm volatile("{\n\t.reg .pred p;\n\tsetp.ne.b32 p, %69, 0;\n\t"
                     "wgmma.mma_async.sync.aligned.m64n128k8.f32.tf32.tf32 {%0, %1, %2, %3, %4, %5, %6, %7, %8, %9, %10, %11, %12, %13, %14, %15, %16, %17, %18, %19, %20, %21, %22, %23, %24, %25, %26, %27, %28, %29, %30, %31, %32, %33, %34, %35, %36, %37, %38, %39, %40, %41, %42, %43, %44, %45, %46, %47, %48, %49, %50, %51, %52, %53, %54, %55, %56, %57, %58, %59, %60, %61, %62, %63}, {%64, %65, %66, %67}, %68, p, 1, 1;\n\t}"
            : "+f"(d[0]), "+f"(d[1]), "+f"(d[2]), "+f"(d[3]), "+f"(d[4]), "+f"(d[5]), "+f"(d[6]), "+f"(d[7]),
              "+f"(d[8]), "+f"(d[9]), "+f"(d[10]), "+f"(d[11]), "+f"(d[12]), "+f"(d[13]), "+f"(d[14]), "+f"(d[15]),
              "+f"(d[16]), "+f"(d[17]), "+f"(d[18]), "+f"(d[19]), "+f"(d[20]), "+f"(d[21]), "+f"(d[22]), "+f"(d[23]),
              "+f"(d[24]), "+f"(d[25]), "+f"(d[26]), "+f"(d[27]), "+f"(d[28]), "+f"(d[29]), "+f"(d[30]), "+f"(d[31]),
              "+f"(d[32]), "+f"(d[33]), "+f"(d[34]), "+f"(d[35]), "+f"(d[36]), "+f"(d[37]), "+f"(d[38]), "+f"(d[39]),
              "+f"(d[40]), "+f"(d[41]), "+f"(d[42]), "+f"(d[43]), "+f"(d[44]), "+f"(d[45]), "+f"(d[46]), "+f"(d[47]),
              "+f"(d[48]), "+f"(d[49]), "+f"(d[50]), "+f"(d[51]), "+f"(d[52]), "+f"(d[53]), "+f"(d[54]), "+f"(d[55]),
              "+f"(d[56]), "+f"(d[57]), "+f"(d[58]), "+f"(d[59]), "+f"(d[60]), "+f"(d[61]), "+f"(d[62]), "+f"(d[63])
            : "r"(a[0]), "r"(a[1]), "r"(a[2]), "r"(a[3]), "l"(db), "r"(acc));
    }
};

}
```

Measured before the change: 3323.

## Add wide 192/256-column wgmma tiles with sliced epilogue and register rebalancing

Adds f16 tap-GEMM kernels with N tile widths of 192 and 256, using m64n192/m64n256 wgmma instructions. They are chosen for large-K convolutions with N of 192 or more, so each A tile loaded through TMA is reused across more output columns. The accumulators now stay in registers through the mainloop, and the epilogue stages them to shared memory in 64-column slices to keep the staging buffer small. setmaxnreg moves registers from the producer warpgroup to the consumers to fit the larger accumulators, at the cost of fewer pipeline stages and more register pressure in the epilogue.

New measurement: 3501 (median of 6 runs). 5.4% higher.

```diff
diff --git a/aero_b200/csrc/tapgemm.cuh b/aero_b200/csrc/tapgemm.cuh
--- a/aero_b200/csrc/tapgemm.cuh
+++ b/aero_b200/csrc/tapgemm.cuh
@@ -29,6 +29,9 @@
 constexpr int kBM = 128;
 constexpr int kMaxStages = 8;
 constexpr int kMaxBN = 128;
+constexpr int kWideBN = 256;
+constexpr int kSliceBN = 64;
+constexpr int kProducerRegs = 40, kConsumerRegs = 232;
 constexpr int kEpiWarps = 8;
 constexpr int kThreads = 128 + 32 * kEpiWarps;
 constexpr int kATileBytes = kBM * 128;
diff --git a/aero_b200/csrc/tapgemm_tc.cu b/aero_b200/csrc/tapgemm_tc.cu
--- a/aero_b200/csrc/tapgemm_tc.cu
+++ b/aero_b200/csrc/tapgemm_tc.cu
@@ -14,6 +14,8 @@
 KernelFn tapgemm_tc_kernels_bn64(bool f16a, bool f16o, int amode, bool res, bool stats);
 KernelFn tapgemm_tc_kernels_bn96(bool f16a, bool f16o, int amode, bool res, bool stats);
 KernelFn tapgemm_tc_kernels_bn128(bool f16a, bool f16o, int amode, bool res, bool stats);
+KernelFn tapgemm_tc_kernels_bn192(bool f16a, bool f16o, int amode, bool res, bool stats);
+KernelFn tapgemm_tc_kernels_bn256(bool f16a, bool f16o, int amode, bool res, bool stats);
 
 typedef CUresult (*EncodeTiledFn)(CUtensorMap*, CUtensorMapDataType, cuuint32_t, void*, const cuuint64_t*, const cuuint64_t*,
                                   const cuuint32_t*, const cuuint32_t*, CUtensorMapInterleave, CUtensorMapSwizzle,
@@ -87,17 +89,30 @@
     return AERO_OK;
 }
 
-static int pick_bn(int N) {
-    const int ntiles = (N + kMaxBN - 1) / kMaxBN;
-    const int per = (N + ntiles - 1) / ntiles;
-    return (per + 31) & ~31;
-}
-
-static int tc_fixed_smem(int N, int BN) { return (int)sizeof(TcShared) + cdiv(N, BN) * BN * 4 + kBM * (BN + 4) * 4 + 1024; }
+static int tc_fixed_smem(int N, int BN) {
+    return (int)sizeof(TcShared) + cdiv(N, BN) * BN * 4 + kBM * ((BN > kMaxBN ? kSliceBN : BN) + 4) * 4 + 1024;
+}
 static int tc_stages(int N, int BN) {
     if (N > (1 << 20)) return 0;
     const int st = (227 * 1024 - tc_fixed_smem(N, BN)) / (kATileBytes + BN * 128);
     return st > kMaxStages ? kMaxStages : st;
+}
+
+constexpr int kWideMinKTaps = 512;
+
+static int pick_bn(const aero_tapgemm_params& p) {
+    const int nt = cdiv(p.N, kMaxBN);
+    const int narrow = (cdiv(p.N, nt) + 31) & ~31;
+    if (p.precision != 2 || p.mode == AERO_TAPS_MIX || p.N < 192) return narrow;
+    const int taps = (p.mode == AERO_TAPS_CONV) ? p.kf * p.kt : p.kf / p.stride_f;
+    if ((int64_t)(p.C1 + p.C2) * taps < kWideMinKTaps) return narrow;
+    const int bn = cdiv(p.N, cdiv(p.N, kWideBN)) <= 192 ? 192 : 256;
+    if (tc_stages(p.N, bn) < 3) return narrow;
+    if (p.stats_mode == 1) {
+        const int Nout = p.glu ? p.N / 2 : p.N;
+        if (p.groups < 1 || Nout % p.groups || (p.glu ? bn / 2 : bn) / (Nout / p.groups) + 2 > 8) return narrow;
+    }
+    return bn;
 }
 
 bool tapgemm_tc_eligible(const aero_tapgemm_params& p) {
@@ -105,12 +120,12 @@
     const int q = f16 ? 8 : 4;
     if (p.mode == AERO_TAPS_MIX)
         return p.w_sb == 0 && p.C1 % q == 0 && p.C2 == 0 && p.a1_st % q == 0 && p.a1_sb % q == 0 && p.N >= 8 &&
-               p.stats_mode == 0 && !p.glu && p.F_out == 1 && p.F_in == 1 && tc_stages(p.N, pick_bn(p.N)) >= 2;
+               p.stats_mode == 0 && !p.glu && p.F_out == 1 && p.F_in == 1 && tc_stages(p.N, pick_bn(p)) >= 2;
     if (p.w_sb != 0) return false;
     if (p.act == AERO_ACT_TANH) return false;
     if (p.act == AERO_ACT_LEAKY && (p.stats_mode != 0 || p.r_sb != 0 || p.r_sf != 0 || p.r_st != 0))
         return false;
-    if (tc_stages(p.N, pick_bn(p.N)) < 2) return false;
+    if (tc_stages(p.N, pick_bn(p)) < 2) return false;
     if (p.N < 8) return false;
     const int K = p.C1 + p.C2;
     if (K < 8 || (p.C1 % q) || (p.C2 % q)) return false;
@@ -121,7 +136,7 @@
         const int Nout = p.glu ? p.N / 2 : p.N;
         if (p.groups < 1 || Nout % p.groups) return false;
         const int gw = Nout / p.groups;
-        const int bn = pick_bn(p.N);
+        const int bn = pick_bn(p);
         if (gw % 8 || (p.glu ? bn / 2 : bn) / gw + 2 > 8) return false;
     }
     return true;
@@ -153,7 +168,7 @@
     const bool f16a = p.precision == 2, f16o = (p.flags & AERO_TG_OUT_F16) != 0;
     const int esz = f16a ? 2 : 4, kBKc = 128 / esz;
     const int K = p.C1 + p.C2;
-    const int BN = pick_bn(p.N);
+    const int BN = pick_bn(p);
     const int nslab = (p.mode == AERO_TAPS_CONVT) ? p.kf : p.kf * p.kt;
     CUtensorMap mA1, mA2, mW;
     int rc;
@@ -207,7 +222,9 @@
     const KernelFn kern = BN == 32 ? tapgemm_tc_kernels_bn32(f16a, f16o, amode, res, stats)
                         : BN == 64 ? tapgemm_tc_kernels_bn64(f16a, f16o, amode, res, stats)
                         : BN == 96 ? tapgemm_tc_kernels_bn96(f16a, f16o, amode, res, stats)
-                                   : tapgemm_tc_kernels_bn128(f16a, f16o, amode, res, stats);
+                        : BN == 128 ? tapgemm_tc_kernels_bn128(f16a, f16o, amode, res, stats)
+                        : BN == 192 ? tapgemm_tc_kernels_bn192(f16a, f16o, amode, res, stats)
+                                    : tapgemm_tc_kernels_bn256(f16a, f16o, amode, res, stats);
     if (!kern) {
         set_error("aero_tapgemm_fwd(wgmma): epilogue (act %d, residual %d, stats %d) is not built for operands %s / outputs %s",
                   amode, (int)res, (int)stats, f16a ? "f16" : "tf32", f16o ? "f16" : "f32");
diff --git a/aero_b200/csrc/tapgemm_tc_bn192.cu b/aero_b200/csrc/tapgemm_tc_bn192.cu
--- /dev/null
+++ b/aero_b200/csrc/tapgemm_tc_bn192.cu
@@ -0,0 +1,5 @@
+#include "tapgemm_tc_kernel.cuh"
+
+namespace aero {
+KernelFn tapgemm_tc_kernels_bn192(bool f16a, bool f16o, int amode, bool res, bool stats) { return pick_kernel_bn<192>(f16a, f16o, amode, res, stats); }
+}
diff --git a/aero_b200/csrc/tapgemm_tc_bn256.cu b/aero_b200/csrc/tapgemm_tc_bn256.cu
--- /dev/null
+++ b/aero_b200/csrc/tapgemm_tc_bn256.cu
@@ -0,0 +1,5 @@
+#include "tapgemm_tc_kernel.cuh"
+
+namespace aero {
+KernelFn tapgemm_tc_kernels_bn256(bool f16a, bool f16o, int amode, bool res, bool stats) { return pick_kernel_bn<256>(f16a, f16o, amode, res, stats); }
+}
diff --git a/aero_b200/csrc/tapgemm_tc_kernel.cuh b/aero_b200/csrc/tapgemm_tc_kernel.cuh
--- a/aero_b200/csrc/tapgemm_tc_kernel.cuh
+++ b/aero_b200/csrc/tapgemm_tc_kernel.cuh
@@ -82,8 +82,8 @@
 }
 
 template <int AMODE, bool RES, bool STATS, typename TO>
-__device__ __forceinline__ void epilogue_fast_tile(TcShared* sh, const TapGemmArgs& g, const TileCoord& tc, uint32_t tacc, int BN, int q,
-                                                   int ew, int lane, int Nout, int gw, int c_start, int c_step, uint32_t sbias) {
+__device__ __forceinline__ void epilogue_fast_tile(TcShared* sh, const TapGemmArgs& g, const TileCoord& tc, uint32_t tacc, int c_lo, int c_hi,
+                                                   int q, int ew, int lane, int Nout, int gw, int c_start, int c_step, uint32_t sbias) {
     const aero_tapgemm_params& p = g.p;
     constexpr int CNT = (AMODE == 3) ? 8 : 16;
     constexpr int LPR = CNT / 4;
@@ -99,12 +99,12 @@
     TO* const obase = static_cast<TO*>(g.out) + (int64_t)tc.b * p.o_sb + (int64_t)tc.fo * p.o_sf + (int64_t)row0 * p.o_st;
     const TO* const rbase = RES ? static_cast<const TO*>(g.residual) + (int64_t)tc.b * p.r_sb + (int64_t)tc.fo * p.r_sf + (int64_t)row0 * p.r_st : nullptr;
     const float* const adp = g.addend_fn ? g.addend_fn + (int64_t)tc.fo * Nout : nullptr;
-    for (int c0 = c_start; c0 < BN; c0 += c_step) {
+    for (int c0 = c_lo + c_start; c0 < c_hi; c0 += c_step) {
         const int nb = tc.n0 + c0;
         if (nb >= p.N) break;
         uint32_t r[16];
         if (tc.n_iters > 0) {
-            acc_ld16(tacc + 4u * (uint32_t)c0, r);
+            acc_ld16(tacc + 4u * (uint32_t)(c0 - c_lo), r);
         } else {
 #pragma unroll
             for (int j = 0; j < 16; ++j) r[j] = 0u;
@@ -170,8 +170,8 @@
 }
 
 template <int AMODE, bool RES, bool STATS, typename TO>
-__device__ __forceinline__ void epilogue_direct(TcShared* sh, const TapGemmArgs& g, const TileCoord& tc, uint32_t tacc, int BN, int q, int ew,
-                                                int lane, int Nout, int gw, int c_start, int c_step, uint32_t sbias) {
+__device__ __forceinline__ void epilogue_direct(TcShared* sh, const TapGemmArgs& g, const TileCoord& tc, uint32_t tacc, int c_lo, int c_hi, int q,
+                                                int ew, int lane, int Nout, int gw, int c_start, int c_step, uint32_t sbias) {
     const aero_tapgemm_params& p = g.p;
     constexpr int CNT = (AMODE == 3) ? 8 : 16;
     constexpr bool F16 = sizeof(TO) == 2;
@@ -187,12 +187,12 @@
     const int g_lo = ((AMODE == 3) ? tc.n0 >> 1 : tc.n0) / gw;
     int cur_g = -1;
     float ssum = 0.f, ssq = 0.f;
-    for (int c0 = c_start; c0 < BN; c0 += c_step) {
+    for (int c0 = c_lo + c_start; c0 < c_hi; c0 += c_step) {
         const int nb = tc.n0 + c0;
         if (nb >= p.N) break;
         uint32_t r[16];
         if (tc.n_iters > 0) {
-            acc_ld16(tacc + 4u * (uint32_t)c0, r);
+            acc_ld16(tacc + 4u * (uint32_t)(c0 - c_lo), r);
         } else {
 #pragma unroll
             for (int j = 0; j < 16; ++j) r[j] = 0u;
@@ -290,8 +290,7 @@
 
 template <int BN, bool F16A>
 __device__ __forceinline__ void tile_mainloop(TcShared* sh, uint8_t* smem, int& stage, uint32_t& phase, const int kStages, const int stage_bytes,
-                                              const int n_iters, const bool mix, const int wg, float* acc, const int ldacc) {
-    float d[BN / 2];
+                                              const int n_iters, const bool mix, const int wg, float (&d)[BN / 2]) {
     const int tid = threadIdx.x & 127, wl = tid >> 5, lane = tid & 31;
     int prev = -1;
     for (int i = 0; i < n_iters; ++i) {
@@ -335,11 +334,18 @@
     }
     wgmma_wait<0>();
     if (prev >= 0 && tid == 0) mbar_arrive(&sh->empty[prev]);
+}
+
+template <int BN, int SW>
+__device__ __forceinline__ void stage_acc(const float (&d)[BN / 2], const int s0, float* acc, const int wg) {
+    constexpr int ldacc = SW + 4;
+    const int tid = threadIdx.x & 127, wl = tid >> 5, lane = tid & 31;
     float* row = acc + (wg * 64 + wl * 16 + (lane >> 2)) * ldacc + 2 * (lane & 3);
 #pragma unroll
-    for (int j = 0; j < BN / 8; ++j) {
-        *reinterpret_cast<float2*>(row + 8 * j) = make_float2(d[4 * j], d[4 * j + 1]);
-        *reinterpret_cast<float2*>(row + 8 * ldacc + 8 * j) = make_float2(d[4 * j + 2], d[4 * j + 3]);
+    for (int j = 0; j < SW / 8; ++j) {
+        const int jd = s0 / 8 + j;
+        *reinterpret_cast<float2*>(row + 8 * j) = make_float2(d[4 * jd], d[4 * jd + 1]);
+        *reinterpret_cast<float2*>(row + 8 * ldacc + 8 * j) = make_float2(d[4 * jd + 2], d[4 * jd + 3]);
     }
 }
 
@@ -354,15 +360,17 @@
     TcShared* sh = reinterpret_cast<TcShared*>(smem + kStages * stage_bytes);
     float* const sbias_f = reinterpret_cast<float*>(sh + 1);
     const uint32_t sbias = smem_u32(sbias_f);
+    constexpr bool kWide = BN > kMaxBN;
+    constexpr int kSW = kWide ? kSliceBN : BN;
     float* const acc = sbias_f + n_tiles * BN;
-    constexpr int ldacc = BN + 4;
+    constexpr int ldacc = kSW + 4;
 
     using TO = typename std::conditional<F16O, __half, float>::type;
     constexpr int kBKc = OperandKind<F16A>::kBK;
     const aero_tapgemm_params& p = g.p;
     const int warp = threadIdx.x >> 5, lane = threadIdx.x & 31;
     const int nch1 = (p.C1 + kBKc - 1) / kBKc, nch2 = (p.C2 + kBKc - 1) / kBKc;
-    const bool mix = p.mode == AERO_TAPS_MIX;
+    const bool mix = !kWide && p.mode == AERO_TAPS_MIX;
 
     for (int i = threadIdx.x; i < n_tiles * BN; i += kThreads) sbias_f[i] = (g.bias && i < g.p.N) ? g.bias[i] : 0.f;
     if (threadIdx.x == 0) {
@@ -373,8 +381,9 @@
     }
     __syncthreads();
 
-    if (warp == 0) {
-        if (lane == 0) {
+    if (warp < 4) {
+        if constexpr (kWide) asm volatile("setmaxnreg.dec.sync.aligned.u32 %0;" ::"n"(kProducerRegs));
+        if (warp == 0 && lane == 0) {
             asm volatile("prefetch.tensormap [%0];" ::"l"(&mapA1) : "memory");
             asm volatile("prefetch.tensormap [%0];" ::"l"(&mapW) : "memory");
             int stage = 0;
@@ -416,7 +425,8 @@
                 }
             }
         }
-    } else if (warp >= 4) {
+    } else {
+        if constexpr (kWide) asm volatile("setmaxnreg.inc.sync.aligned.u32 %0;" ::"n"(kConsumerRegs));
         const int wg = (warp >> 2) - 1;
         const int ew = warp - 4;
         const int q = 2 * wg + (warp & 1);
@@ -432,121 +442,127 @@
         for (int tile = blockIdx.x; tile < tiles_total; tile += gridDim.x, ++local) {
             const TileCoord tc = tile_coord(g, tile, n_tiles, BN, nch1, nch2);
             const int b = tc.b, fo = tc.fo, t0 = tc.t0, n0 = tc.n0, n_iters = tc.n_iters;
-            tile_mainloop<BN, F16A>(sh, smem, stage, phase, kStages, stage_bytes, n_iters, mix, wg, acc, ldacc);
-            warpgroup_sync(1 + wg);
-            const uint32_t tacc = smem_u32(acc + m * ldacc);
-            const int t = t0 + m;
-            const bool row_ok = t < p.T;
-            float sa = 1.f, sb = 0.f;
-            if (g.samp_affine) { sa = g.samp_affine[2 * b]; sb = g.samp_affine[2 * b + 1]; }
-            TO* op = static_cast<TO*>(g.out) + (int64_t)b * p.o_sb + (int64_t)fo * p.o_sf + (int64_t)t * p.o_st;
-            const TO* rp = g.residual ? static_cast<const TO*>(g.residual) + (int64_t)b * p.r_sb + (int64_t)fo * p.r_sf + (int64_t)t * p.r_st : nullptr;
-            const float* csp = g.colscale ? g.colscale + (int64_t)b * p.cs_sb + (int64_t)t * p.cs_st : nullptr;
-            const float* adp = g.addend_fn ? g.addend_fn + (int64_t)fo * Nout : nullptr;
-            int cur_g = -1;
-            float ssum = 0.f, ssq = 0.f;
             const int g_lo = (p.glu ? n0 >> 1 : n0) / gw;
-
-            if (mix) {
-                const float gate = (row_ok && g.colscale) ? g.colscale[(int64_t)b * p.cs_sb + t] : 1.f;
-                TO* ob = static_cast<TO*>(g.out) + (int64_t)b * p.o_sb + t;
-                for (int c0 = c_start; c0 < BN; c0 += c_step) {
-                    uint32_t r[16];
-                    acc_ld16(tacc + 4u * (uint32_t)c0, r);
-                    if (row_ok) {
+            float d[BN / 2];
+            tile_mainloop<BN, F16A>(sh, smem, stage, phase, kStages, stage_bytes, n_iters, mix, wg, d);
+#pragma unroll
+            for (int s0 = 0; s0 < BN; s0 += kSW) {
+                if (s0 > 0) warpgroup_sync(1 + wg);
+                stage_acc<BN, kSW>(d, s0, acc, wg);
+                warpgroup_sync(1 + wg);
+                const uint32_t tacc = smem_u32(acc + m * ldacc);
+                const int t = t0 + m;
+                const bool row_ok = t < p.T;
+                float sa = 1.f, sb = 0.f;
+                if (g.samp_affine) { sa = g.samp_affine[2 * b]; sb = g.samp_affine[2 * b + 1]; }
+                TO* op = static_cast<TO*>(g.out) + (int64_t)b * p.o_sb + (int64_t)fo * p.o_sf + (int64_t)t * p.o_st;
+                const TO* rp = g.residual ? static_cast<const TO*>(g.residual) + (int64_t)b * p.r_sb + (int64_t)fo * p.r_sf + (int64_t)t * p.r_st : nullptr;
+                const float* csp = g.colscale ? g.colscale + (int64_t)b * p.cs_sb + (int64_t)t * p.cs_st : nullptr;
+                const float* adp = g.addend_fn ? g.addend_fn + (int64_t)fo * Nout : nullptr;
+                int cur_g = -1;
+                float ssum = 0.f, ssq = 0.f;
+
+                if (mix) {
+                    const float gate = (row_ok && g.colscale) ? g.colscale[(int64_t)b * p.cs_sb + t] : 1.f;
+                    TO* ob = static_cast<TO*>(g.out) + (int64_t)b * p.o_sb + t;
+                    for (int c0 = c_start; c0 < BN; c0 += c_step) {
+                        uint32_t r[16];
+                        acc_ld16(tacc + 4u * (uint32_t)c0, r);
+                        if (row_ok) {
+#pragma unroll
+                            for (int j = 0; j < 16; ++j) {
+                                const int n = n0 + c0 + j;
+                                if (n < p.N) {
+                                    float x = __uint_as_float(r[j]) * gate;
+                                    if (rnd) x = round_tf32_rna(x);
+                                    stf(ob + (int64_t)n * p.o_st, x);
+                                }
+                            }
+                        }
+                    }
+                } else if (fast && (F16O ? (g.vec_o8 && (g.direct_f16 == 1 || (g.direct_f16 == 2 && AMODE == 3))) : g.direct_f32)) {
+                    epilogue_direct<AMODE, RES, STATS, TO>(sh, g, tc, tacc, s0, s0 + kSW, q, ew, lane, Nout, gw, c_start, c_step, sbias);
+                } else if (fast) {
+                    epilogue_fast_tile<AMODE, RES, STATS, TO>(sh, g, tc, tacc, s0, s0 + kSW, q, ew, lane, Nout, gw, c_start, c_step, sbias);
+                } else {
+                    for (int c0 = s0; c0 < (grp == 0 ? s0 + kSW : s0); c0 += 16) {
+                        uint32_t r[16];
+                        if (n_iters > 0) {
+                            acc_ld16(tacc + 4u * (uint32_t)(c0 - s0), r);
+                        } else {
+#pragma unroll
+                            for (int j = 0; j < 16; ++j) r[j] = 0u;
+                        }
+                        const int nb = n0 + c0;
+                        if (nb >= p.N) continue;
+                        float v[16];
 #pragma unroll
                         for (int j = 0; j < 16; ++j) {
-                            const int n = n0 + c0 + j;
-                            if (n < p.N) {
-                                float x = __uint_as_float(r[j]) * gate;
-                                if (rnd) x = round_tf32_rna(x);
-                                stf(ob + (int64_t)n * p.o_st, x);
+                            const int n = nb + j;
+                            float x = __uint_as_float(r[j]);
+                            if (row_ok && n < p.N) {
+                                x += sbias_f[n];
+                                if (csp) x *= csp[n];
+                                if (p.act == AERO_ACT_GELU) x = gelu_exact(x);
+                                else if (p.act == AERO_ACT_RELU) x = fmaxf(x, 0.f);
+                                else if (AMODE == 4) x = leaky_f(x);
                             }
-                        }
-                    }
-                }
-            } else if (fast && (F16O ? (g.vec_o8 && (g.direct_f16 == 1 || (g.direct_f16 == 2 && AMODE == 3))) : g.direct_f32)) {
-                epilogue_direct<AMODE, RES, STATS, TO>(sh, g, tc, tacc, BN, q, ew, lane, Nout, gw, c_start, c_step, sbias);
-            } else if (fast) {
-                epilogue_fast_tile<AMODE, RES, STATS, TO>(sh, g, tc, tacc, BN, q, ew, lane, Nout, gw, c_start, c_step, sbias);
-            } else {
-                for (int c0 = 0; c0 < (grp == 0 ? BN : 0); c0 += 16) {
-                    uint32_t r[16];
-                    if (n_iters > 0) {
-                        acc_ld16(tacc + 4u * (uint32_t)c0, r);
-                    } else {
-#pragma unroll
-                        for (int j = 0; j < 16; ++j) r[j] = 0u;
-                    }
-                    const int nb = n0 + c0;
-                    if (nb >= p.N) continue;
-                    float v[16];
-#pragma unroll
-                    for (int j = 0; j < 16; ++j) {
-                        const int n = nb + j;
-                        float x = __uint_as_float(r[j]);
-                        if (row_ok && n < p.N) {
-                            x += sbias_f[n];
-                            if (csp) x *= csp[n];
-                            if (p.act == AERO_ACT_GELU) x = gelu_exact(x);
-                            else if (p.act == AERO_ACT_RELU) x = fmaxf(x, 0.f);
-                            else if (AMODE == 4) x = leaky_f(x);
-                        }
-                        v[j] = x;
-                    }
-                    float o[16];
-                    int no0, cnt;
-                    if (p.glu) {
-                        no0 = nb >> 1;
-                        cnt = 8;
-#pragma unroll
-                        for (int j = 0; j < 8; ++j) o[j] = v[2 * j] * sigmoid_f(v[2 * j + 1]);
-                    } else {
-                        no0 = nb;
-                        cnt = 16;
-#pragma unroll
-                        for (int j = 0; j < 16; ++j) o[j] = v[j];
-                    }
-#pragma unroll
-                    for (int sub = 0; sub < 2; ++sub) {
-                        if (sub * 8 >= cnt) break;
-                        const int ns = no0 + sub * 8;
-                        if (p.stats_mode != 0 && ns < Nout) {
-                            const int gi = ns / gw;
-                            if (gi != cur_g) {
-                                if (cur_g >= 0) {
-                                    const float a = warp_sum(ssum), c = warp_sum(ssq);
-                                    if (lane == 0) { sh->stats[ew][cur_g - g_lo][0] = a; sh->stats[ew][cur_g - g_lo][1] = c; }
+                            v[j] = x;
+                        }
+                        float o[16];
+                        int no0, cnt;
+                        if (p.glu) {
+                            no0 = nb >> 1;
+                            cnt = 8;
+#pragma unroll
+                            for (int j = 0; j < 8; ++j) o[j] = v[2 * j] * sigmoid_f(v[2 * j + 1]);
+                        } else {
+                            no0 = nb;
+                            cnt = 16;
+#pragma unroll
+                            for (int j = 0; j < 16; ++j) o[j] = v[j];
+                        }
+#pragma unroll
+                        for (int sub = 0; sub < 2; ++sub) {
+                            if (sub * 8 >= cnt) break;
+                            const int ns = no0 + sub * 8;
+                            if (p.stats_mode != 0 && ns < Nout) {
+                                const int gi = ns / gw;
+                                if (gi != cur_g) {
+                                    if (cur_g >= 0) {
+                                        const float a = warp_sum(ssum), c = warp_sum(ssq);
+                                        if (lane == 0) { sh->stats[ew][cur_g - g_lo][0] += a; sh->stats[ew][cur_g - g_lo][1] += c; }
+                                    }
+                                    cur_g = gi; ssum = 0.f; ssq = 0.f;
                                 }
-                                cur_g = gi; ssum = 0.f; ssq = 0.f;
                             }
-                        }
-#pragma unroll
-                        for (int j = 0; j < 8; ++j) {
-                            const int jj = sub * 8 + j;
-                            const int nn = no0 + jj;
-                            if (row_ok && nn < Nout) {
-                                float x = o[jj];
-                                if (adp) x += adp[nn];
-                                if (rp) x += ldf(rp + nn);
-                                x = x * sa + sb;
-                                if (rnd) x = round_tf32_rna(x);
-                                x = stored(x, op);
-                                o[jj] = x;
-                                ssum += x;
-                                ssq += x * x;
+#pragma unroll
+                            for (int j = 0; j < 8; ++j) {
+                                const int jj = sub * 8 + j;
+                                const int nn = no0 + jj;
+                                if (row_ok && nn < Nout) {
+                                    float x = o[jj];
+                                    if (adp) x += adp[nn];
+                                    if (rp) x += ldf(rp + nn);
+                                    x = x * sa + sb;
+                                    if (rnd) x = round_tf32_rna(x);
+                                    x = stored(x, op);
+                                    o[jj] = x;
+                                    ssum += x;
+                                    ssq += x * x;
+                                }
                             }
                         }
-                    }
-                    if (row_ok) {
-#pragma unroll
-                        for (int j = 0; j < 16; ++j)
-                            if (j < cnt && no0 + j < Nout) stf(op + no0 + j, o[j]);
-                    }
-                }
-                if (p.stats_mode != 0 && cur_g >= 0) {
-                    const float a = warp_sum(ssum), c = warp_sum(ssq);
-                    if (lane == 0) { sh->stats[ew][cur_g - g_lo][0] = a; sh->stats[ew][cur_g - g_lo][1] = c; }
+                        if (row_ok) {
+#pragma unroll
+                            for (int j = 0; j < 16; ++j)
+                                if (j < cnt && no0 + j < Nout) stf(op + no0 + j, o[j]);
+                        }
+                    }
+                    if (p.stats_mode != 0 && cur_g >= 0) {
+                        const float a = warp_sum(ssum), c = warp_sum(ssq);
+                        if (lane == 0) { sh->stats[ew][cur_g - g_lo][0] += a; sh->stats[ew][cur_g - g_lo][1] += c; }
+                    }
                 }
             }
             warpgroup_sync(1 + wg);
@@ -607,8 +623,11 @@
 
 template <int BN>
 static KernelFn pick_kernel_bn(bool f16a, bool f16o, int amode, bool res, bool stats) {
-    return f16a ? (f16o ? pick_kernel<BN, true, true>(amode, res, stats) : pick_kernel<BN, true, false>(amode, res, stats))
-                : (f16o ? pick_kernel<BN, false, true>(amode, res, stats) : pick_kernel<BN, false, false>(amode, res, stats));
-}
-
-}
+    if constexpr (BN > kMaxBN)
+        return !f16a ? nullptr : f16o ? pick_kernel<BN, true, true>(amode, res, stats) : pick_kernel<BN, true, false>(amode, res, stats);
+    else
+        return f16a ? (f16o ? pick_kernel<BN, true, true>(amode, res, stats) : pick_kernel<BN, true, false>(amode, res, stats))
+                    : (f16o ? pick_kernel<BN, false, true>(amode, res, stats) : pick_kernel<BN, false, false>(amode, res, stats));
+}
+
+}
diff --git a/aero_b200/csrc/wgmma.cuh b/aero_b200/csrc/wgmma.cuh
--- a/aero_b200/csrc/wgmma.cuh
+++ b/aero_b200/csrc/wgmma.cuh
@@ -285,4 +285,48 @@
     }
 };
 
+template <int TA> struct Wgmma<192, true, TA> {
+    static __device__ __forceinline__ void ss(float (&d)[96], uint64_t da, uint64_t db, uint32_t acc) {
+        asm volatile("{\n\t.reg .pred p;\n\tsetp.ne.b32 p, %98, 0;\n\t"
+                     "wgmma.mma_async.sync.aligned.m64n192k16.f32.f16.f16 {%0, %1, %2, %3, %4, %5, %6, %7, %8, %9, %10, %11, %12, %13, %14, %15, %16, %17, %18, %19, %20, %21, %22, %23, %24, %25, %26, %27, %28, %29, %30, %31, %32, %33, %34, %35, %36, %37, %38, %39, %40, %41, %42, %43, %44, %45, %46, %47, %48, %49, %50, %51, %52, %53, %54, %55, %56, %57, %58, %59, %60, %61, %62, %63, %64, %65, %66, %67, %68, %69, %70, %71, %72, %73, %74, %75, %76, %77, %78, %79, %80, %81, %82, %83, %84, %85, %86, %87, %88, %89, %90, %91, %92, %93, %94, %95}, %96, %97, p, 1, 1, %99, 0;\n\t}"
+            : "+f"(d[0]), "+f"(d[1]), "+f"(d[2]), "+f"(d[3]), "+f"(d[4]), "+f"(d[5]), "+f"(d[6]), "+f"(d[7]),
+              "+f"(d[8]), "+f"(d[9]), "+f"(d[10]), "+f"(d[11]), "+f"(d[12]), "+f"(d[13]), "+f"(d[14]), "+f"(d[15]),
+              "+f"(d[16]), "+f"(d[17]), "+f"(d[18]), "+f"(d[19]), "+f"(d[20]), "+f"(d[21]), "+f"(d[22]), "+f"(d[23]),
+              "+f"(d[24]), "+f"(d[25]), "+f"(d[26]), "+f"(d[27]), "+f"(d[28]), "+f"(d[29]), "+f"(d[30]), "+f"(d[31]),
+              "+f"(d[32]), "+f"(d[33]), "+f"(d[34]), "+f"(d[35]), "+f"(d[36]), "+f"(d[37]), "+f"(d[38]), "+f"(d[39]),
+              "+f"(d[40]), "+f"(d[41]), "+f"(d[42]), "+f"(d[43]), "+f"(d[44]), "+f"(d[45]), "+f"(d[46]), "+f"(d[47]),
+              "+f"(d[48]), "+f"(d[49]), "+f"(d[50]), "+f"(d[51]), "+f"(d[52]), "+f"(d[53]), "+f"(d[54]), "+f"(d[55]),
+              "+f"(d[56]), "+f"(d[57]), "+f"(d[58]), "+f"(d[59]), "+f"(d[60]), "+f"(d[61]), "+f"(d[62]), "+f"(d[63]),
+              "+f"(d[64]), "+f"(d[65]), "+f"(d[66]), "+f"(d[67]), "+f"(d[68]), "+f"(d[69]), "+f"(d[70]), "+f"(d[71]),
+              "+f"(d[72]), "+f"(d[73]), "+f"(d[74]), "+f"(d[75]), "+f"(d[76]), "+f"(d[77]), "+f"(d[78]), "+f"(d[79]),
+              "+f"(d[80]), "+f"(d[81]), "+f"(d[82]), "+f"(d[83]), "+f"(d[84]), "+f"(d[85]), "+f"(d[86]), "+f"(d[87]),
+              "+f"(d[88]), "+f"(d[89]), "+f"(d[90]), "+f"(d[91]), "+f"(d[92]), "+f"(d[93]), "+f"(d[94]), "+f"(d[95])
+            : "l"(da), "l"(db), "r"(acc), "n"(TA));
+    }
+};
+
+template <int TA> struct Wgmma<256, true, TA> {
+    static __device__ __forceinline__ void ss(float (&d)[128], uint64_t da, uint64_t db, uint32_t acc) {
+        asm volatile("{\n\t.reg .pred p;\n\tsetp.ne.b32 p, %130, 0;\n\t"
+                     "wgmma.mma_async.sync.aligned.m64n256k16.f32.f16.f16 {%0, %1, %2, %3, %4, %5, %6, %7, %8, %9, %10, %11, %12, %13, %14, %15, %16, %17, %18, %19, %20, %21, %22, %23, %24, %25, %26, %27, %28, %29, %30, %31, %32, %33, %34, %35, %36, %37, %38, %39, %40, %41, %42, %43, %44, %45, %46, %47, %48, %49, %50, %51, %52, %53, %54, %55, %56, %57, %58, %59, %60, %61, %62, %63, %64, %65, %66, %67, %68, %69, %70, %71, %72, %73, %74, %75, %76, %77, %78, %79, %80, %81, %82, %83, %84, %85, %86, %87, %88, %89, %90, %91, %92, %93, %94, %95, %96, %97, %98, %99, %100, %101, %102, %103, %104, %105, %106, %107, %108, %109, %110, %111, %112, %113, %114, %115, %116, %117, %118, %119, %120, %121, %122, %123, %124, %125, %126, %127}, %128, %129, p, 1, 1, %131, 0;\n\t}"
+            : "+f"(d[0]), "+f"(d[1]), "+f"(d[2]), "+f"(d[3]), "+f"(d[4]), "+f"(d[5]), "+f"(d[6]), "+f"(d[7]),
+              "+f"(d[8]), "+f"(d[9]), "+f"(d[10]), "+f"(d[11]), "+f"(d[12]), "+f"(d[13]), "+f"(d[14]), "+f"(d[15]),
+              "+f"(d[16]), "+f"(d[17]), "+f"(d[18]), "+f"(d[19]), "+f"(d[20]), "+f"(d[21]), "+f"(d[22]), "+f"(d[23]),
+              "+f"(d[24]), "+f"(d[25]), "+f"(d[26]), "+f"(d[27]), "+f"(d[28]), "+f"(d[29]), "+f"(d[30]), "+f"(d[31]),
+              "+f"(d[32]), "+f"(d[33]), "+f"(d[34]), "+f"(d[35]), "+f"(d[36]), "+f"(d[37]), "+f"(d[38]), "+f"(d[39]),
+              "+f"(d[40]), "+f"(d[41]), "+f"(d[42]), "+f"(d[43]), "+f"(d[44]), "+f"(d[45]), "+f"(d[46]), "+f"(d[47]),
+              "+f"(d[48]), "+f"(d[49]), "+f"(d[50]), "+f"(d[51]), "+f"(d[52]), "+f"(d[53]), "+f"(d[54]), "+f"(d[55]),
+              "+f"(d[56]), "+f"(d[57]), "+f"(d[58]), "+f"(d[59]), "+f"(d[60]), "+f"(d[61]), "+f"(d[62]), "+f"(d[63]),
+              "+f"(d[64]), "+f"(d[65]), "+f"(d[66]), "+f"(d[67]), "+f"(d[68]), "+f"(d[69]), "+f"(d[70]), "+f"(d[71]),
+              "+f"(d[72]), "+f"(d[73]), "+f"(d[74]), "+f"(d[75]), "+f"(d[76]), "+f"(d[77]), "+f"(d[78]), "+f"(d[79]),
+              "+f"(d[80]), "+f"(d[81]), "+f"(d[82]), "+f"(d[83]), "+f"(d[84]), "+f"(d[85]), "+f"(d[86]), "+f"(d[87]),
+              "+f"(d[88]), "+f"(d[89]), "+f"(d[90]), "+f"(d[91]), "+f"(d[92]), "+f"(d[93]), "+f"(d[94]), "+f"(d[95]),
+              "+f"(d[96]), "+f"(d[97]), "+f"(d[98]), "+f"(d[99]), "+f"(d[100]), "+f"(d[101]), "+f"(d[102]), "+f"(d[103]),
+              "+f"(d[104]), "+f"(d[105]), "+f"(d[106]), "+f"(d[107]), "+f"(d[108]), "+f"(d[109]), "+f"(d[110]), "+f"(d[111]),
+              "+f"(d[112]), "+f"(d[113]), "+f"(d[114]), "+f"(d[115]), "+f"(d[116]), "+f"(d[117]), "+f"(d[118]), "+f"(d[119]),
+              "+f"(d[120]), "+f"(d[121]), "+f"(d[122]), "+f"(d[123]), "+f"(d[124]), "+f"(d[125]), "+f"(d[126]), "+f"(d[127])
+            : "l"(da), "l"(db), "r"(acc), "n"(TA));
+    }
+};
+
 }
```
